# ericbill21/map-dit

Hardware: AMD Instinct MI355X
Metric: latent-images/sec training step, DiT-B/2 bf16 @256 (higher is better)
Workload: dtype bf16; 1 GPU; DiT-B/2 full training step on 32x32x4 latents (fresh batch+fwd+loss+bwd+grad reduction+Adam+2xEMA), all magnitude-preserving features on, bf16 GEMM operands / fp32 accumulate, master and residual fp32; global_batch=256, per_gpu_batch=256, parallelism=dp1, grad_comm=allreduce-fp32-per-stage-overlapped

## Files before the change

include/mapdit.h:

```cpp
#ifndef MAPDIT_H
#define MAPDIT_H

#include <stddef.h>
#include <stdint.h>

#ifdef __cplusplus
extern "C" {
#endif

#define MAPDIT_OK 0
#define MAPDIT_ERR_ARG 1
#define MAPDIT_ERR_HIP 2

const char* mapdit_last_error(void);
int mapdit_abi_version(void);

enum { MAPDIT_NT = 0, MAPDIT_NN = 1, MAPDIT_TN = 2 };

enum {
    MAPDIT_EPI_STORE_BF16 = 0,
    MAPDIT_EPI_STORE_F32 = 1,
    MAPDIT_EPI_SILU2 = 2,
    MAPDIT_EPI_RESID = 3,
    MAPDIT_EPI_DSILU = 4,
    MAPDIT_EPI_SILU2_COND = 5,
    MAPDIT_EPI_SILU2_GRAD = 7,
    MAPDIT_EPI_MUL_AUX = 8,
    MAPDIT_EPI_RMB = 9,
    MAPDIT_EPI_QKV_HEADS = 6,
    MAPDIT_EPI_QKV_HEADS_RAW = 10
};

typedef struct {
    int kind;
    void* out;
    int ldo;
    void* out2;
    const void* aux;
    const float* gate;
    int ldg;
    int rows_per_sample;
    float alpha, beta;
    int accumulate;
    void* out3;
    const float* shift2;
    const float* scale2;
    const float* gain2;
    int ld2;
    int split_k;
    long slab_stride;
    void* out4;
    const void* rmb;
    int rot2;
} mapdit_epilogue_t;

int mapdit_gemm_bf16(int layout, int M, int N, int K, const uint16_t* A, int lda, const uint16_t* B, int ldb,
                     const mapdit_epilogue_t* epi, void* stream);
typedef struct {
    const uint16_t* A; int lda;
    const uint16_t* B; int ldb;
    int M, N;
    float* out; int ldo;
    float alpha;
    long slab_stride;
} mapdit_gemm_group_item_t;
int mapdit_gemm_group_tn_bf16(int n, const mapdit_gemm_group_item_t* items, int K, int split_k, void* stream);
int mapdit_gemm_tile_size(int M, int N);
int mapdit_gemm_tile_size_ex(int M, int N, int split_k_launch);
int mapdit_gemm_tile_size_k(int M, int N, int K, int split_k_launch);
void mapdit_gemm_tuning(int tile, int phases, long band);

enum { MAPDIT_WN_PLAIN = 2 };
int mapdit_weightnorm_fwd(float* W, int rows, int cols, int forced, float out_scale, uint16_t* w_bf16, float* w_f32,
                          float* inv, void* stream);
typedef struct {
    float* W;
    int rows, cols;
    float out_scale;
    int first_block;
    uint16_t* w_bf16;
    float* w_f32;
    uint16_t* w_split3;
    int flags;
} mapdit_wn_job_t;
int mapdit_weightnorm_fwd_batch(const mapdit_wn_job_t* jobs_dev, int njobs, int total_blocks, int forced, void* stream);
int mapdit_weightnorm_bwd(const float* W, float* G, int ldg, int nslabs, long slab_stride, float* dW, int rows,
                          int cols, float out_scale, int accumulate, void* stream);
int mapdit_weightnorm_bwd_batch(const mapdit_wn_job_t* jobs_dev, int njobs, int total_blocks, void* stream);
typedef struct {
    const float* W; float* G; int ldg; int nslabs; long slab_stride; float* dW; int rows, cols; float out_scale; int flags;
} mapdit_wn_bwd_item_t;
int mapdit_weightnorm_bwd_group(int n, const mapdit_wn_bwd_item_t* items, void* stream);
int mapdit_weightnorm_bwd_slim(const float* W, float* G, int ldg, int nslabs, long slab_stride, float* dW, int rows,
                               int cols, float out_scale, int accumulate, void* stream);

typedef struct {
    long lo, hi, first_block;
} mapdit_range_t;

int mapdit_adam_ema_step(float* params, const float* grads, float* exp_avg, float* exp_avg_sq, float* ema_a,
                         float* ema_b, long n, const float* hyper, float beta1, float beta2, float eps, void* stream);
typedef struct {
    float step_size;
    float inv_sqrt_bc2;
    float ema_beta_a, ema_beta_b;
    float grad_scale;
} mapdit_adam_scalars_t;
int mapdit_adam_ema_step_scalars(float* params, const float* grads, float* exp_avg, float* exp_avg_sq, float* ema_a,
                                 float* ema_b, long n, const mapdit_adam_scalars_t* hyper, float beta1, float beta2,
                                 float eps, void* stream);
int mapdit_grad_nonfinite_check(const float* grads, long n, int* status, int step, void* stream);
int mapdit_adam_ema_step_guarded(float* params, const float* grads, float* exp_avg, float* exp_avg_sq, float* ema_a, float* ema_b,
                                 long n, const mapdit_adam_scalars_t* hyper, float beta1, float beta2, float eps,
                                 const int* status, int step, void* stream);
int mapdit_adam_ema_step_ranges(float* params, const float* grads, float* exp_avg, float* exp_avg_sq, float* ema_a, float* ema_b,
                                const mapdit_range_t* ranges_dev, int nranges, long total_blocks, const mapdit_adam_scalars_t* hyper,
                                float beta1, float beta2, float eps, const int* status, int step, void* stream);
int mapdit_grad_nonfinite_check_ranges(const float* grads, const mapdit_range_t* ranges_dev, int nranges, long total_blocks, int* status,
                                       int step, void* stream);

int mapdit_modulate_fwd(const float* x, const float* shift, const float* scale, int ldmod, const float* gain,
                        uint16_t* out, int n_samples, int T, int D, void* stream);

int mapdit_ln_modulate_fwd(const float* x, const float* shift, const float* scale, int ldmod, const float* gain, float* xhat, float* rstd,
                           uint16_t* out, int n_samples, int T, int D, void* stream);
int mapdit_ln_bwd_merge(const float* dxhat, const float* xhat, const float* rstd, const float* dxo, const uint16_t* dxo16, float ca, float* out,
                        long rows, int D, void* stream);

typedef struct {
    const float* dxo;
    const uint16_t* dxm;
    const float* x;
    const float* shift;
    const float* scale;
    const float* gain;
    const uint16_t* y_up;
    const float* g_up;
    float* dx;
    uint16_t* dx_bf;
    float* dshift;
    float* dscale;
    float* dgain_part;
    uint16_t* dy_up;
    float* dg_up;
    int ldmod, ldg_up, ldd, ldd_up;
    int n_samples, T, D;
    float ca, cb;
    float* part_scratch;
    size_t part_scratch_bytes;
    int* gain_partials_out;
    float* dgain_out;
    int rot;
    float dgain_scale;
    const uint16_t* dxo_bf;
    int ldx;
} mapdit_resid_mod_bwd_t;
int mapdit_resid_mod_bwd(const mapdit_resid_mod_bwd_t* args, void* stream);

int mapdit_rot_coef_fwd(const float* theta, const float* scale, int ldm, const float* gain, float* A, float* B, int ldc,
                        int n_samples, int D, void* stream);
#define MAPDIT_ROT_MAX_SLOTS 80
int mapdit_rot_coef_fwd_all(const float* mod, int ld_mod, const int* theta_off, const int* scale_off, const float* const* gains,
                            int n_slots, float* A, float* B, int ldc, int n_samples, int D, void* stream);
int mapdit_rot_coef_bwd(const float* dA, const float* dB, int ldc, const float* theta, const float* scale, int ldm,
                        const float* gain, float* dtheta, float* dscale, int ldd, float* dgain_part, float dgain_scale,
                        int n_samples, int D, void* stream);
int mapdit_rot_modulate_fwd(const float* x, const float* A, const float* B, int ldc, uint16_t* out, int n_samples, int T, int D,
                            void* stream);
int mapdit_reduce_partials(const float* part, int count, float* out, int accumulate, void* stream);

int mapdit_mpsilu_to_bf16(const float* x, uint16_t* out, long n, void* stream);
int mapdit_f32_to_bf16(const float* x, uint16_t* out, long n, float alpha, void* stream);
int mapdit_f32_to_bf16_2d(const float* x, int ldx, uint16_t* out, int ldo, int rows, int cols, float alpha, void* stream);
int mapdit_sum_slabs(float* acc, const float* slabs, int nslabs, long slab_stride, long n, void* stream);
int mapdit_reduce_slabs(float* out, const float* slabs, int nslabs, long slab_stride, long n, void* stream);
int mapdit_reduce_slabs_group(int n, float* const* outs, const float* const* slabs, const long* slab_strides, const long* ns, int nslabs, void* stream);
int mapdit_sum_bf16_chunks(float* out, const uint16_t* chunks, int nchunks, long chunk_stride, long n, void* stream);
int mapdit_scale_copy(float* out, const float* x, long n, float alpha, void* stream);

int mapdit_qkv_split(const uint16_t* qkv, int B, int T, int H, int head_dim, uint16_t* qn, uint16_t* kn, uint16_t* v,
                     void* stream);
int mapdit_qkv_merge_bwd(const uint16_t* qkv, int B, int T, int H, int head_dim, const uint16_t* dqn,
                         const uint16_t* dkn, const uint16_t* dv, uint16_t* dqkv, void* stream);
int mapdit_attn_cos_fwd(const uint16_t* qn, const uint16_t* kn, const uint16_t* v, uint16_t* o, float* lse, int B,
                        int T, int H, int head_dim, void* stream);
int mapdit_attn_cos_fwd_rawqk(const uint16_t* q, const uint16_t* k, const uint16_t* v, uint16_t* o, float* lse, int B, int T, int H,
                              int head_dim, void* stream);
int mapdit_attn_cos_fwd_rawqk_save(uint16_t* q, uint16_t* k, const uint16_t* v, uint16_t* o, float* lse, float* scales, int B, int T,
                                   int H, int head_dim, void* stream);
int mapdit_qk_cos_normalize(uint16_t* q, uint16_t* k, float* scales, int B, int T, int H, int head_dim, void* stream);
int mapdit_attn_sdpa_fwd(const uint16_t* q, const uint16_t* k, const uint16_t* v, uint16_t* o, float* lse, int B, int T, int H,
                         int head_dim, void* stream);
int mapdit_heads_merge_bwd(const uint16_t* dqn, const uint16_t* dkn, const uint16_t* dv, int B, int T, int H, int head_dim, uint16_t* dqkv,
                           void* stream);
int mapdit_attn_cos_bwd(const uint16_t* qn, const uint16_t* kn, const uint16_t* v, const uint16_t* dO, const uint16_t* O,
                        const float* lse, float* delta, uint16_t* dqn, uint16_t* dkn, uint16_t* dv, int B, int T, int H,
                        int head_dim, void* stream);
int mapdit_attn_cos_bwd_fused(const uint16_t* qn, const uint16_t* kn, const uint16_t* v, const uint16_t* dO, const uint16_t* O,
                              const float* lse, float* delta, const float* scales, uint16_t* dqkv, int B, int T, int H,
                              int head_dim, void* stream);

int mapdit_qkv_split_generic(const uint16_t* qkv, int B, int T, int H, int head_dim, uint16_t* qn, uint16_t* kn, uint16_t* v,
                             void* stream);
int mapdit_qkv_merge_bwd_generic(const uint16_t* qkv, int B, int T, int H, int head_dim, const uint16_t* dqn,
                                 const uint16_t* dkn, const uint16_t* dv, uint16_t* dqkv, void* stream);
int mapdit_attn_generic_fwd(const uint16_t* qn, const uint16_t* kn, const uint16_t* v, uint16_t* o, float* lse, int B, int T,
                            int H, int head_dim, void* stream);
int mapdit_attn_generic_bwd(const uint16_t* qn, const uint16_t* kn, const uint16_t* v, const uint16_t* dO, const uint16_t* O,
                            const float* lse, float* delta, uint16_t* dqn, uint16_t* dkn, uint16_t* dv, int B, int T, int H,
                            int head_dim, void* stream);

int mapdit_patch_embed_fwd(const float* x, const float* w_eff, const float* pos, float* out, uint16_t* patches,
                           int ldp, int N, int C, int S, int p, int D, float out_scale, void* stream);
int mapdit_patch_embed_bwd_x(const uint16_t* dx0, int ldx, const float* w_eff, float* dx, int N, int C, int S, int p, int D, float scale,
                             void* stream);
int mapdit_fourier_fwd(const int64_t* t, const float* scale, const float* shift, uint16_t* out, int n, int F,
                       void* stream);
int mapdit_cond_combine_fwd(const float* temb, const float* table, const int64_t* y, float* c, uint16_t* c_silu,
                            uint16_t* c_bf, int n, int D, int table_rows, void* stream);
int mapdit_cond_combine_bwd(const float* c, const float* dcs, const float* dcd, const int64_t* y, uint16_t* dtemb,
                            float* dtable, int n, int D, int table_rows, void* stream);
int mapdit_device_error_poll(void* stream);
int mapdit_final_out_fwd(const float* lin, int ldl, const float* a_mean, const float* a_sigma, const float* ref_mean,
                         const float* ref_sigma, float* out, int N, int C, int S, int p, void* stream);
int mapdit_final_out_bwd(const float* dout, const float* lin, int ldl, const float* a_mean, const float* a_sigma,
                         const float* ref_mean, const float* ref_sigma, uint16_t* dlin, int ldd, uint16_t* da_bf,
                         float* dref_part , float* dref_mean , float* dref_sigma,
                         float grad_scale, int N, int C, int S, int p, void* stream);
int mapdit_cfg_combine(const float* model_out, float* out, int n_total, int C, int HW, float cfg_scale, void* stream);
int mapdit_cfg_combine_bwd(const float* dout, float* din, int n_total, int C, int HW, float cfg_scale, void* stream);

int mapdit_q_sample(const float* x0, const float* noise, const int64_t* t, const float* tab, int nsteps, float* xt,
                    int N, int per_sample, void* stream);
int mapdit_loss_fwd(const float* model_out, const float* x0, const float* xt, const float* noise, const int64_t* t,
                    const float* tab, int nsteps, float* mse, float* vb, float* loss, float* G, int N, int per_sample,
                    void* stream);
int mapdit_loss_bwd(const float* G, const float* g_loss, const float* g_mse, const float* g_vb, float* dout, int N,
                    int per_sample, void* stream);
int mapdit_psample_step(const float* model_out, const float* x, const float* noise, const int64_t* t, const float* tab,
                        int nsteps, int clip_denoised, float* sample, float* pred_xstart, int N, int per_sample,
                        void* stream);
int mapdit_ddim_step(const float* model_out, const float* x, const float* noise, const int64_t* t, const float* tab,
                     const float* dtab, int nsteps, int clip_denoised, float eta, int reverse, float* sample, float* pred_xstart,
                     int N, int per_sample, void* stream);

int mapdit_obj_loss_fwd(const float* model_out, const float* x0, const float* xt, const float* noise, const int64_t* t,
                        const float* tab, const float* otab, int nsteps, int mean_type, int var_type, int loss_type, float* mse,
                        float* vb, float* loss, float* G, int N, int per_sample, void* stream);
int mapdit_obj_loss_bwd(const float* G, const float* g_loss, const float* g_mse, const float* g_vb, float* dout, int N,
                        int per_sample, int groups, void* stream);
int mapdit_obj_step(const float* model_out, const float* x, const float* noise, const int64_t* t, const float* tab,
                    const float* otab, int nsteps, int mean_type, int var_type, int clip_denoised, int mode, float eta,
                    float* sample, float* pred_xstart, int N, int per_sample, void* stream);
int mapdit_obj_xstart(const float* model_out, const float* x, const int64_t* t, const float* tab, int nsteps, int mean_type,
                      int var_type, float* xstart, int N, int per_sample, void* stream);
int mapdit_obj_step_guided(const float* model_out, const float* x, const float* noise, const int64_t* t, const float* tab,
                           const float* otab, int nsteps, int mean_type, int var_type, int clip_denoised, int mode, float eta,
                           const float* xstart_in, const float* cond_grad, float* sample, float* pred_xstart, float* mean, int N,
                           int per_sample, void* stream);
int mapdit_dpm_step(const float* model_out, const float* x, float* hist, const int64_t* step, const float* ctab, const int64_t* tau,
                    int K, const float* tab, int nsteps, int mean_type, int var_type, int clip_denoised, const float* xstart_in,
                    float* sample, float* pred_xstart, int N, int per_sample, void* stream);
int mapdit_obj_vb_terms(const float* model_out, const float* x0, const float* xt, const float* noise, const int64_t* t,
                        const float* tab, const float* otab, int nsteps, int mean_type, int var_type, int clip_denoised, float* vb,
                        float* xstart_mse, float* mse, float* pred_xstart, int ld, int col_from_t, int N, int per_sample,
                        void* stream);
int mapdit_prior_bpd(const float* x0, const float* tab, const float* otab, int nsteps, const float* vb, float* prior, float* total,
                     int N, int per_sample, void* stream);

enum { MAPDIT_OFF_MP_SILU = 1, MAPDIT_OFF_MP_RESIDUAL = 2, MAPDIT_OFF_MP_POS_ENC = 4, MAPDIT_OFF_MP_EMBEDDING = 8,
       MAPDIT_OFF_WEIGHT_NORM = 16, MAPDIT_OFF_COSINE_ATTN = 32, MAPDIT_OFF_NO_LAYERNORM = 64 };
typedef struct {
    int depth, hidden, patch, input_size, in_channels, num_heads, mlp_hidden;
    int table_rows;
    int max_batch;
    int precision;
    int rotation;
    int mp_off;
    float loss_scale;
    int recompute;
} mapdit_config_t;
enum { MAPDIT_RECOMPUTE_NONE = 0, MAPDIT_RECOMPUTE_MLP = 1, MAPDIT_RECOMPUTE_BLOCK = 2 };
enum { MAPDIT_PREC_BF16 = 0, MAPDIT_PREC_BF16X3 = 1, MAPDIT_PREC_F16 = 2 };

enum {
    MAPDIT_P_X_EMB = 0, MAPDIT_P_T0, MAPDIT_P_T2, MAPDIT_P_Y_EMB, MAPDIT_P_F_LIN, MAPDIT_P_F_MOD, MAPDIT_P_MS_LIN,
    MAPDIT_P_MS_REF, MAPDIT_P_SS_LIN, MAPDIT_P_SS_REF, MAPDIT_P_F_GAIN, MAPDIT_P_FOURIER_SCALE, MAPDIT_P_FOURIER_SHIFT,
    MAPDIT_P_POS_EMBED, MAPDIT_NUM_GLOBAL
};
enum { MAPDIT_B_QKV = 0, MAPDIT_B_PROJ, MAPDIT_B_FC1, MAPDIT_B_FC2, MAPDIT_B_MOD, MAPDIT_B_GAIN_MSA, MAPDIT_B_GAIN_MLP, MAPDIT_NUM_BLOCK };

typedef struct mapdit_engine mapdit_engine_t;

size_t mapdit_engine_workspace_bytes(const mapdit_config_t* cfg, int train);
int mapdit_engine_create(const mapdit_config_t* cfg, int train, void* workspace, size_t workspace_bytes, void* stream,
                         mapdit_engine_t** out);
void mapdit_engine_destroy(mapdit_engine_t* e);
int mapdit_engine_bind(mapdit_engine_t* e, float* const* params_host, float* const* grads_host);
int mapdit_engine_prepare_weights(mapdit_engine_t* e, int forced, void* stream);
int mapdit_engine_forward(mapdit_engine_t* e, const float* x, const int64_t* t, const int64_t* y_eff, int N, int save,
                          float* out, void* stream);
int mapdit_engine_backward(mapdit_engine_t* e, const float* dout, void* stream);
int mapdit_engine_backward_stages(mapdit_engine_t* e, const float* dout, int stage_from, int stage_to, void* stream);
int mapdit_engine_set_shard(mapdit_engine_t* e, int rank, int world);
int mapdit_engine_set_block_fences(mapdit_engine_t* e, void* const* events, int n);
int mapdit_engine_weight_image(mapdit_engine_t* e, int pidx, void** img, void** img3, int* rows, int* cols, int* sharded);
int mapdit_engine_jacobian_shard(mapdit_engine_t* e, void* stream);
int mapdit_engine_set_loss_scale(mapdit_engine_t* e, float loss_scale);
int mapdit_engine_loss_scale(mapdit_engine_t* e, float* out);
int mapdit_engine_set_input_grad(mapdit_engine_t* e, float* dx, int input_only);

enum { MAPDIT_PROF_FC1_FWD = 0 };
int mapdit_engine_profile_begin(mapdit_engine_t* e, int which, int max_events);
int mapdit_engine_profile_begin_strided(mapdit_engine_t* e, int which, int max_events, int stride);
int mapdit_engine_profile_end(mapdit_engine_t* e, int* count, double* total_ms);

enum { MAPDIT_PEEK_G_FOUR = 0, MAPDIT_PEEK_G_TEMB, MAPDIT_PEEK_G_C, MAPDIT_PEEK_G_MOD_ALL, MAPDIT_PEEK_G_X0, MAPDIT_PEEK_G_XMODF,
       MAPDIT_PEEK_G_LIN, MAPDIT_PEEK_B_XM, MAPDIT_PEEK_B_QKV, MAPDIT_PEEK_B_QN, MAPDIT_PEEK_B_KN, MAPDIT_PEEK_B_V, MAPDIT_PEEK_B_O,
       MAPDIT_PEEK_B_XM2, MAPDIT_PEEK_B_HACT, MAPDIT_PEEK_B_XMID, MAPDIT_PEEK_B_XOUT, MAPDIT_PEEK_COUNT };
int mapdit_engine_peek(mapdit_engine_t* e, int what, int block, void** ptr, long* elems, int* ld, int* dtype);

typedef struct mapdit_comm mapdit_comm_t;
int mapdit_comm_unique_id(void* id128);
int mapdit_comm_create(const void* id128, int rank, int world, mapdit_comm_t** out);
void mapdit_comm_destroy(mapdit_comm_t* comm);
int mapdit_allreduce_bucket(mapdit_comm_t* comm, float* buf, long count, void* stream);
int mapdit_reduce_scatter_bucket(mapdit_comm_t* comm, float* buf, long count, void* stream);
int mapdit_allgather_bucket(mapdit_comm_t* comm, float* buf, long count, void* stream);

int mapdit_gemm_f16(int layout, int M, int N, int K, const uint16_t* A, int lda, const uint16_t* B, int ldb,
                    const mapdit_epilogue_t* epi, void* stream);
int mapdit_gemm_group_tn_f16(int n, const mapdit_gemm_group_item_t* items, int K, int split_k, void* stream);
int mapdit_weightnorm_fwd_f16(float* W, int rows, int cols, int forced, float out_scale, uint16_t* w_f16, float* w_f32,
                              float* inv, void* stream);
int mapdit_weightnorm_fwd_batch_f16(const mapdit_wn_job_t* jobs_dev, int njobs, int total_blocks, int forced, void* stream);
int mapdit_modulate_fwd_f16(const float* x, const float* shift, const float* scale, int ldmod, const float* gain,
                            uint16_t* out, int n_samples, int T, int D, void* stream);
int mapdit_resid_mod_bwd_f16(const mapdit_resid_mod_bwd_t* args, void* stream);
int mapdit_ln_modulate_fwd_f16(const float* x, const float* shift, const float* scale, int ldmod, const float* gain, float* xhat, float* rstd,
                               uint16_t* out, int n_samples, int T, int D, void* stream);
int mapdit_ln_bwd_merge_f16(const float* dxhat, const float* xhat, const float* rstd, const float* dxo, const uint16_t* dxo16, float ca, float* out,
                            long rows, int D, void* stream);
int mapdit_rot_modulate_fwd_f16(const float* x, const float* A, const float* B, int ldc, uint16_t* out, int n_samples, int T, int D,
                                void* stream);
int mapdit_mpsilu_to_f16(const float* x, uint16_t* out, long n, void* stream);
int mapdit_f32_to_f16(const float* x, uint16_t* out, long n, float alpha, void* stream);
int mapdit_f32_to_f16_2d(const float* x, int ldx, uint16_t* out, int ldo, int rows, int cols, float alpha, void* stream);
int mapdit_qkv_split_f16(const uint16_t* qkv, int B, int T, int H, int head_dim, uint16_t* qn, uint16_t* kn, uint16_t* v,
                         void* stream);
int mapdit_qkv_merge_bwd_f16(const uint16_t* qkv, int B, int T, int H, int head_dim, const uint16_t* dqn,
                             const uint16_t* dkn, const uint16_t* dv, uint16_t* dqkv, void* stream);
int mapdit_attn_cos_fwd_f16(const uint16_t* qn, const uint16_t* kn, const uint16_t* v, uint16_t* o, float* lse, int B,
                            int T, int H, int head_dim, void* stream);
int mapdit_attn_cos_fwd_rawqk_f16(const uint16_t* q, const uint16_t* k, const uint16_t* v, uint16_t* o, float* lse, int B, int T, int H,
                                  int head_dim, void* stream);
int mapdit_attn_cos_fwd_rawqk_save_f16(uint16_t* q, uint16_t* k, const uint16_t* v, uint16_t* o, float* lse, float* scales, int B, int T,
                                       int H, int head_dim, void* stream);
int mapdit_qk_cos_normalize_f16(uint16_t* q, uint16_t* k, float* scales, int B, int T, int H, int head_dim, void* stream);
int mapdit_attn_sdpa_fwd_f16(const uint16_t* q, const uint16_t* k, const uint16_t* v, uint16_t* o, float* lse, int B, int T, int H,
                             int head_dim, void* stream);
int mapdit_heads_merge_bwd_f16(const uint16_t* dqn, const uint16_t* dkn, const uint16_t* dv, int B, int T, int H, int head_dim, uint16_t* dqkv,
                               void* stream);
int mapdit_attn_cos_bwd_f16(const uint16_t* qn, const uint16_t* kn, const uint16_t* v, const uint16_t* dO, const uint16_t* O,
                            const float* lse, float* delta, uint16_t* dqn, uint16_t* dkn, uint16_t* dv, int B, int T, int H,
                            int head_dim, void* stream);
int mapdit_attn_cos_bwd_fused_f16(const uint16_t* qn, const uint16_t* kn, const uint16_t* v, const uint16_t* dO, const uint16_t* O,
                                  const float* lse, float* delta, const float* scales, uint16_t* dqkv, int B, int T, int H,
                                  int head_dim, void* stream);
int mapdit_qkv_split_generic_f16(const uint16_t* qkv, int B, int T, int H, int head_dim, uint16_t* qn, uint16_t* kn, uint16_t* v,
                                 void* stream);
int mapdit_qkv_merge_bwd_generic_f16(const uint16_t* qkv, int B, int T, int H, int head_dim, const uint16_t* dqn,
                                     const uint16_t* dkn, const uint16_t* dv, uint16_t* dqkv, void* stream);
int mapdit_attn_generic_fwd_f16(const uint16_t* qn, const uint16_t* kn, const uint16_t* v, uint16_t* o, float* lse, int B, int T,
                                int H, int head_dim, void* stream);
int mapdit_attn_generic_bwd_f16(const uint16_t* qn, const uint16_t* kn, const uint16_t* v, const uint16_t* dO, const uint16_t* O,
                                const float* lse, float* delta, uint16_t* dqn, uint16_t* dkn, uint16_t* dv, int B, int T, int H,
                                int head_dim, void* stream);
int mapdit_patch_embed_fwd_f16(const float* x, const float* w_eff, const float* pos, float* out, uint16_t* patches,
                               int ldp, int N, int C, int S, int p, int D, float out_scale, void* stream);
int mapdit_patch_embed_bwd_x_f16(const uint16_t* dx0, int ldx, const float* w_eff, float* dx, int N, int C, int S, int p, int D, float scale,
                                 void* stream);
int mapdit_cond_combine_fwd_f16(const float* temb, const float* table, const int64_t* y, float* c, uint16_t* c_silu,
                                uint16_t* c_f16, int n, int D, int table_rows, void* stream);
int mapdit_cond_combine_bwd_f16(const float* c, const float* dcs, const float* dcd, const int64_t* y, uint16_t* dtemb,
                                float* dtable, int n, int D, int table_rows, void* stream);
int mapdit_final_out_bwd_f16(const float* dout, const float* lin, int ldl, const float* a_mean, const float* a_sigma,
                             const float* ref_mean, const float* ref_sigma, uint16_t* dlin, int ldd, uint16_t* da_f16,
                             float* dref_part, float* dref_mean, float* dref_sigma, float grad_scale, int N, int C, int S, int p,
                             void* stream);

#ifdef __cplusplus
}
#endif
#endif
```

map-dit_amd/_lib.py:

```python
from __future__ import annotations

import ctypes as C
import os
import subprocess
import threading

_HERE = os.path.dirname(os.path.abspath(__file__))
LIB_PATH = os.environ.get("MAPDIT_LIB") or os.path.join(_HERE, "libmapdit_hip.so")
CSRC = os.path.join(_HERE, "csrc")

vp, ci, cf, cl = C.c_void_p, C.c_int, C.c_float, C.c_long


class MapditError(RuntimeError):
    pass


class Epilogue(C.Structure):
    _fields_ = [("kind", ci), ("out", vp), ("ldo", ci), ("out2", vp), ("aux", vp), ("gate", vp), ("ldg", ci),
                ("rows_per_sample", ci), ("alpha", cf), ("beta", cf), ("accumulate", ci), ("out3", vp), ("shift2", vp), ("scale2", vp),
                ("gain2", vp), ("ld2", ci), ("split_k", ci), ("slab_stride", cl), ("out4", vp), ("rmb", vp), ("rot2", ci)]


class ResidModBwd(C.Structure):
    _fields_ = [("dxo", vp), ("dxm", vp), ("x", vp), ("shift", vp), ("scale", vp), ("gain", vp), ("y_up", vp),
                ("g_up", vp), ("dx", vp), ("dx_bf", vp), ("dshift", vp), ("dscale", vp), ("dgain_part", vp),
                ("dy_up", vp), ("dg_up", vp), ("ldmod", ci), ("ldg_up", ci), ("ldd", ci), ("ldd_up", ci),
                ("n_samples", ci), ("T", ci), ("D", ci), ("ca", cf), ("cb", cf), ("part_scratch", vp), ("part_scratch_bytes", C.c_size_t),
                ("gain_partials_out", C.POINTER(ci)), ("dgain_out", vp), ("rot", ci), ("dgain_scale", cf), ("dxo_bf", vp), ("ldx", ci)]


class GemmGroupItem(C.Structure):
    _fields_ = [("A", vp), ("lda", ci), ("B", vp), ("ldb", ci), ("M", ci), ("N", ci), ("out", vp), ("ldo", ci), ("alpha", cf), ("slab_stride", cl)]


class WnBwdItem(C.Structure):
    _fields_ = [("W", vp), ("G", vp), ("ldg", ci), ("nslabs", ci), ("slab_stride", cl), ("dW", vp), ("rows", ci), ("cols", ci), ("out_scale", cf),
                ("flags", ci)]


class WnJob(C.Structure):
    _fields_ = [("W", vp), ("rows", ci), ("cols", ci), ("out_scale", cf), ("first_block", ci), ("w_bf16", vp), ("w_f32", vp),
                ("w_split3", vp), ("flags", ci)]


class AdamScalars(C.Structure):
    _fields_ = [("step_size", cf), ("inv_sqrt_bc2", cf), ("ema_beta_a", cf), ("ema_beta_b", cf), ("grad_scale", cf)]


class Config(C.Structure):
    _fields_ = [("depth", ci), ("hidden", ci), ("patch", ci), ("input_size", ci), ("in_channels", ci),
                ("num_heads", ci), ("mlp_hidden", ci), ("table_rows", ci), ("max_batch", ci), ("precision", ci), ("rotation", ci),
                ("mp_off", ci), ("loss_scale", cf), ("recompute", ci)]


MP_OFF = {"mp_silu": 1, "mp_residual": 2, "mp_pos_enc": 4, "mp_embedding": 8, "weight_normalization": 16, "cosine_attention": 32, "no_layernorm": 64}
WN_PLAIN = 2


PRECISIONS = {"bf16": 0, "bf16x3": 1, "f16": 2}

RECOMPUTE = {"none": 0, "mlp": 1, "block": 2}


NT, NN, TN = 0, 1, 2
EPI_STORE_BF16, EPI_STORE_F32, EPI_SILU2, EPI_RESID, EPI_DSILU, EPI_SILU2_COND, EPI_QKV_HEADS, EPI_SILU2_GRAD, EPI_MUL_AUX, EPI_RMB, EPI_QKV_HEADS_RAW = range(11)
PROF_FC1_FWD = 0
PEEK_IDS = {name: i for i, name in enumerate(
    ["four", "temb", "c", "mod_all", "x0", "xmodf", "lin", "xm", "qkv", "qn", "kn", "v", "o", "xm2", "hact", "xmid", "xout"])}

(P_X_EMB, P_T0, P_T2, P_Y_EMB, P_F_LIN, P_F_MOD, P_MS_LIN, P_MS_REF, P_SS_LIN, P_SS_REF, P_F_GAIN, P_FOURIER_SCALE,
 P_FOURIER_SHIFT, P_POS_EMBED, NUM_GLOBAL) = range(15)
(B_QKV, B_PROJ, B_FC1, B_FC2, B_MOD, B_GAIN_MSA, B_GAIN_MLP, NUM_BLOCK) = range(8)

_SIGS = {
    "mapdit_gemm_bf16": [ci, ci, ci, ci, vp, ci, vp, ci, C.POINTER(Epilogue), vp],
    "mapdit_gemm_group_tn_bf16": [ci, vp, ci, ci, vp],
    "mapdit_weightnorm_fwd": [vp, ci, ci, ci, cf, vp, vp, vp, vp],
    "mapdit_weightnorm_bwd": [vp, vp, ci, ci, cl, vp, ci, ci, cf, ci, vp],
    "mapdit_weightnorm_bwd_slim": [vp, vp, ci, ci, cl, vp, ci, ci, cf, ci, vp],
    "mapdit_weightnorm_bwd_batch": [vp, ci, ci, vp],
    "mapdit_weightnorm_bwd_group": [ci, vp, vp],
    "mapdit_reduce_slabs_group": [ci, vp, vp, vp, vp, ci, vp],
    "mapdit_weightnorm_fwd_batch": [vp, ci, ci, ci, vp],
    "mapdit_adam_ema_step": [vp, vp, vp, vp, vp, vp, cl, vp, cf, cf, cf, vp],
    "mapdit_adam_ema_step_scalars": [vp, vp, vp, vp, vp, vp, cl, C.POINTER(AdamScalars), cf, cf, cf, vp],
    "mapdit_adam_ema_step_guarded": [vp, vp, vp, vp, vp, vp, cl, C.POINTER(AdamScalars), cf, cf, cf, vp, ci, vp],
    "mapdit_grad_nonfinite_check": [vp, cl, vp, ci, vp],
    "mapdit_adam_ema_step_ranges": [vp, vp, vp, vp, vp, vp, vp, ci, cl, C.POINTER(AdamScalars), cf, cf, cf, vp, ci, vp],
    "mapdit_grad_nonfinite_check_ranges": [vp, vp, ci, cl, vp, ci, vp],
    "mapdit_modulate_fwd": [vp, vp, vp, ci, vp, vp, ci, ci, ci, vp],
    "mapdit_resid_mod_bwd": [C.POINTER(ResidModBwd), vp],
    "mapdit_reduce_partials": [vp, ci, vp, ci, vp],
    "mapdit_rot_coef_fwd": [vp, vp, ci, vp, vp, vp, ci, ci, ci, vp],
    "mapdit_rot_coef_fwd_all": [vp, ci, vp, vp, vp, ci, vp, vp, ci, ci, ci, vp],
    "mapdit_rot_coef_bwd": [vp, vp, ci, vp, vp, ci, vp, vp, vp, ci, vp, cf, ci, ci, vp],
    "mapdit_rot_modulate_fwd": [vp, vp, vp, ci, vp, ci, ci, ci, vp],
    "mapdit_mpsilu_to_bf16": [vp, vp, cl, vp],
    "mapdit_f32_to_bf16": [vp, vp, cl, cf, vp],
    "mapdit_f32_to_bf16_2d": [vp, ci, vp, ci, ci, ci, cf, vp],
    "mapdit_sum_slabs": [vp, vp, ci, cl, cl, vp],
    "mapdit_scale_copy": [vp, vp, cl, cf, vp],
    "mapdit_reduce_slabs": [vp, vp, ci, cl, cl, vp],
    "mapdit_sum_bf16_chunks": [vp, vp, ci, cl, cl, vp],
    "mapdit_qkv_split": [vp, ci, ci, ci, ci, vp, vp, vp, vp],
    "mapdit_qkv_merge_bwd": [vp, ci, ci, ci, ci, vp, vp, vp, vp, vp],
    "mapdit_attn_cos_fwd": [vp, vp, vp, vp, vp, ci, ci, ci, ci, vp],
    "mapdit_attn_sdpa_fwd": [vp, vp, vp, vp, vp, ci, ci, ci, ci, vp],
    "mapdit_ln_modulate_fwd": [vp, vp, vp, ci, vp, vp, vp, vp, ci, ci, ci, vp],
    "mapdit_ln_bwd_merge": [vp, vp, vp, vp, vp, cf, vp, cl, ci, vp],
    "mapdit_heads_merge_bwd": [vp, vp, vp, ci, ci, ci, ci, vp, vp],
    "mapdit_attn_cos_fwd_rawqk": [vp, vp, vp, vp, vp, ci, ci, ci, ci, vp],
    "mapdit_attn_cos_fwd_rawqk_save": [vp, vp, vp, vp, vp, vp, ci, ci, ci, ci, vp],
    "mapdit_qk_cos_normalize": [vp, vp, vp, ci, ci, ci, ci, vp],
    "mapdit_attn_cos_bwd": [vp] * 10 + [ci, ci, ci, ci, vp],
    "mapdit_attn_cos_bwd_fused": [vp] * 9 + [ci, ci, ci, ci, vp],
    "mapdit_qkv_split_generic": [vp, ci, ci, ci, ci, vp, vp, vp, vp],
    "mapdit_qkv_merge_bwd_generic": [vp, ci, ci, ci, ci, vp, vp, vp, vp, vp],
    "mapdit_attn_generic_fwd": [vp, vp, vp, vp, vp, ci, ci, ci, ci, vp],
    "mapdit_attn_generic_bwd": [vp] * 10 + [ci, ci, ci, ci, vp],
    "mapdit_patch_embed_fwd": [vp, vp, vp, vp, vp, ci, ci, ci, ci, ci, ci, cf, vp],
    "mapdit_patch_embed_bwd_x": [vp, ci, vp, vp, ci, ci, ci, ci, ci, cf, vp],
    "mapdit_fourier_fwd": [vp, vp, vp, vp, ci, ci, vp],
    "mapdit_cond_combine_fwd": [vp, vp, vp, vp, vp, vp, ci, ci, ci, vp],
    "mapdit_cond_combine_bwd": [vp, vp, vp, vp, vp, vp, ci, ci, ci, vp],
    "mapdit_device_error_poll": [vp],
    "mapdit_comm_unique_id": [vp],
    "mapdit_comm_create": [vp, ci, ci, C.POINTER(vp)],
    "mapdit_allreduce_bucket": [vp, vp, cl, vp],
    "mapdit_reduce_scatter_bucket": [vp, vp, cl, vp],
    "mapdit_allgather_bucket": [vp, vp, cl, vp],
    "mapdit_final_out_fwd": [vp, ci, vp, vp, vp, vp, vp, ci, ci, ci, ci, vp],
    "mapdit_final_out_bwd": [vp, vp, ci, vp, vp, vp, vp, vp, ci, vp, vp, vp, vp, cf, ci, ci, ci, ci, vp],
    "mapdit_cfg_combine": [vp, vp, ci, ci, ci, cf, vp],
    "mapdit_cfg_combine_bwd": [vp, vp, ci, ci, ci, cf, vp],
    "mapdit_q_sample": [vp, vp, vp, vp, ci, vp, ci, ci, vp],
    "mapdit_loss_fwd": [vp, vp, vp, vp, vp, vp, ci, vp, vp, vp, vp, ci, ci, vp],
    "mapdit_loss_bwd": [vp, vp, vp, vp, vp, ci, ci, vp],
    "mapdit_psample_step": [vp, vp, vp, vp, vp, ci, ci, vp, vp, ci, ci, vp],
    "mapdit_ddim_step": [vp, vp, vp, vp, vp, vp, ci, ci, cf, ci, vp, vp, ci, ci, vp],
    "mapdit_obj_loss_fwd": [vp, vp, vp, vp, vp, vp, vp, ci, ci, ci, ci, vp, vp, vp, vp, ci, ci, vp],
    "mapdit_obj_loss_bwd": [vp, vp, vp, vp, vp, ci, ci, ci, vp],
    "mapdit_obj_step": [vp, vp, vp, vp, vp, vp, ci, ci, ci, ci, ci, cf, vp, vp, ci, ci, vp],
    "mapdit_obj_xstart": [vp, vp, vp, vp, ci, ci, ci, vp, ci, ci, vp],
    "mapdit_obj_step_guided": [vp, vp, vp, vp, vp, vp, ci, ci, ci, ci, ci, cf, vp, vp, vp, vp, vp, ci, ci, vp],
    "mapdit_dpm_step": [vp, vp, vp, vp, vp, vp, ci, vp, ci, ci, ci, ci, vp, vp, vp, ci, ci, vp],
    "mapdit_obj_vb_terms": [vp, vp, vp, vp, vp, vp, vp, ci, ci, ci, ci, vp, vp, vp, vp, ci, ci, ci, ci, vp],
    "mapdit_prior_bpd": [vp, vp, vp, ci, vp, vp, vp, ci, ci, vp],
    "mapdit_engine_create": [C.POINTER(Config), ci, vp, C.c_size_t, vp, C.POINTER(vp)],
    "mapdit_engine_bind": [vp, C.POINTER(vp), C.POINTER(vp)],
    "mapdit_engine_prepare_weights": [vp, ci, vp],
    "mapdit_engine_forward": [vp, vp, vp, vp, ci, ci, vp, vp],
    "mapdit_engine_backward": [vp, vp, vp],
    "mapdit_engine_backward_stages": [vp, vp, ci, ci, vp],
    "mapdit_engine_set_shard": [vp, ci, ci],
    "mapdit_engine_set_block_fences": [vp, C.POINTER(vp), ci],
    "mapdit_engine_weight_image": [vp, ci, C.POINTER(vp), C.POINTER(vp), C.POINTER(ci), C.POINTER(ci), C.POINTER(ci)],
    "mapdit_engine_jacobian_shard": [vp, vp],
    "mapdit_engine_set_loss_scale": [vp, cf],
    "mapdit_engine_loss_scale": [vp, C.POINTER(cf)],
    "mapdit_engine_set_input_grad": [vp, vp, ci],
    "mapdit_engine_profile_begin": [vp, ci, ci],
    "mapdit_engine_profile_begin_strided": [vp, ci, ci, ci],
    "mapdit_engine_profile_end": [vp, C.POINTER(ci), C.POINTER(C.c_double)],
    "mapdit_engine_peek": [vp, ci, ci, C.POINTER(vp), C.POINTER(C.c_long), C.POINTER(ci), C.POINTER(ci)],
}
for _n in ("weightnorm_fwd", "weightnorm_fwd_batch", "modulate_fwd", "resid_mod_bwd", "rot_modulate_fwd", "qkv_split",
           "qkv_merge_bwd", "attn_cos_fwd", "attn_cos_fwd_rawqk", "attn_cos_fwd_rawqk_save", "qk_cos_normalize", "attn_cos_bwd", "attn_cos_bwd_fused", "attn_sdpa_fwd", "heads_merge_bwd", "ln_modulate_fwd", "ln_bwd_merge", "qkv_split_generic", "qkv_merge_bwd_generic",
           "attn_generic_fwd", "attn_generic_bwd", "patch_embed_fwd", "patch_embed_bwd_x", "cond_combine_fwd", "cond_combine_bwd", "final_out_bwd"):
    _SIGS[f"mapdit_{_n}_f16"] = _SIGS[f"mapdit_{_n}"]
for _b, _h in (("gemm_bf16", "gemm_f16"), ("gemm_group_tn_bf16", "gemm_group_tn_f16"), ("f32_to_bf16", "f32_to_f16"), ("f32_to_bf16_2d", "f32_to_f16_2d"),
               ("mpsilu_to_bf16", "mpsilu_to_f16")):
    _SIGS[f"mapdit_{_h}"] = _SIGS[f"mapdit_{_b}"]
_OTHER = {
    "mapdit_last_error": (C.c_char_p, []),
    "mapdit_abi_version": (ci, []),
    "mapdit_gemm_tile_size": (ci, [ci, ci]),
    "mapdit_gemm_tile_size_ex": (ci, [ci, ci, ci]),
    "mapdit_gemm_tile_size_k": (ci, [ci, ci, ci, ci]),
    "mapdit_gemm_tuning": (None, [ci, ci, cl]),
    "mapdit_engine_workspace_bytes": (C.c_size_t, [C.POINTER(Config), ci]),
    "mapdit_engine_destroy": (None, [vp]),
    "mapdit_comm_destroy": (None, [vp]),
}
EXPORTS = sorted(list(_SIGS) + list(_OTHER))

_lock = threading.Lock()
_handle = None


def _source_digest() -> str:
    import hashlib
    h = hashlib.sha256()
    inc = os.path.join(os.path.dirname(_HERE), "include", "mapdit.h")
    files = sorted(os.path.join(CSRC, f) for f in os.listdir(CSRC) if f.endswith((".hip", ".h")) or f == "Makefile") + [inc]
    for f in files:
        h.update(os.path.basename(f).encode() + b"\0")
        with open(f, "rb") as fh:
            h.update(fh.read())
    return h.hexdigest()


def build(force: bool = False) -> str:
    stamp = LIB_PATH + ".src-sha256"
    digest = _source_digest()
    if not force and os.path.exists(LIB_PATH) and os.path.exists(stamp) and open(stamp).read().strip() == digest:
        return LIB_PATH
    if force:
        subprocess.check_call(["make", "-C", CSRC, "clean"])
    subprocess.check_call(["make", "-C", CSRC, "-j8"])
    with open(stamp, "w") as f:
        f.write(digest + "\n")
    return LIB_PATH


class _Lib:
    def __init__(self, cdll):
        self._cdll = cdll
        for name, argtypes in _SIGS.items():
            fn = getattr(cdll, name)
            fn.argtypes = argtypes
            fn.restype = ci
            setattr(self, name[len("mapdit_"):], self._wrap(name, fn))
        for name, (res, argtypes) in _OTHER.items():
            fn = getattr(cdll, name)
            fn.argtypes = argtypes
            fn.restype = res
            setattr(self, name[len("mapdit_"):], fn)

    def _wrap(self, name, fn):
        def call(*args):
            rc = fn(*args)
            if rc != 0:
                raise MapditError(f"{name} failed ({rc}): {self._cdll.mapdit_last_error().decode()}")
        call.__name__ = name
        return call


def lib() -> _Lib:
    global _handle
    with _lock:
        if _handle is None:
            if not os.path.exists(LIB_PATH):
                raise MapditError(f"{LIB_PATH} is missing: run `python -c 'import __graft_entry__ as g; g.build()'` "
                                  f"or `make -C {CSRC}`; there is no CPU fallback")
            import torch
            _handle = _Lib(C.CDLL(LIB_PATH))
        return _handle


def ptr(t):
    return None if t is None else t.data_ptr()


def cur_stream():
    import torch
    return torch.cuda.current_stream().cuda_stream
```

map-dit_amd/csrc/gemm.hip:

```cpp
#include <stdarg.h>
#include <type_traits>
#include <stdio.h>

#include "common.h"

MD_NS_OPEN

constexpr int BM = 128, BN = 128, BKT = 64;
constexpr int TILE_BYTES = 16384;
constexpr int BUF_BYTES = 2 * TILE_BYTES;
constexpr int CS_LD = 132;
constexpr int SMEM_BYTES = BM * CS_LD * 4;

enum { OP_ROW = 0, OP_KMAJ = 1 };

struct GemmP {
    const bf16_t* A;
    const bf16_t* B;
    int lda, ldb;
    int M, N, K;
    int tiles_n;
    int tiles;
    int split_k;
    int band;
    int phases;
    int n_off;
    int stagger;
};

__device__ __forceinline__ int kswz(int k) { return (k & 3) | ((k >> 1) & 4); }

__device__ __attribute__((aligned(16))) const unsigned int g_zero16[4] = {0u, 0u, 0u, 0u};

template <int KIND, bool KTAIL>
__device__ __forceinline__ void stage_tile(const bf16_t* __restrict__ G, int ld, int idx0, int idx_max, int k0, int kmax,
                                           char* tile, int wave, int lane) {
#pragma unroll
    for (int j = 0; j < 4; ++j) {
        const int seg = wave * 4 + j;
        const bf16_t* src;
        if (KIND == OP_ROW) {
            const int row = seg * 8 + (lane >> 3);
            const int c = (lane & 7) ^ (row & 7);
            int grow = idx0 + row;
            grow = grow < idx_max ? grow : idx_max - 1;
            src = G + (size_t)grow * ld + k0 + c * 8;
            if (KTAIL && k0 + c * 8 >= kmax) src = (const bf16_t*)g_zero16;
        } else {
            const int krow = seg * 4 + (lane >> 4);
            const int c = (lane & 15) ^ (kswz(krow) << 1);
            int col = idx0 + c * 8;
            col = col < idx_max ? col : 0;
            src = G + (size_t)(k0 + krow) * ld + col;
            if (KTAIL && k0 + krow >= kmax) src = (const bf16_t*)g_zero16;
        }
        __builtin_amdgcn_global_load_lds(src, (lds_void_t*)(tile + seg * 1024), 16, 0, 0);
    }
}

template <int KIND, bool TR_ASM = true>
__device__ __forceinline__ bf16x8_t read_frag(const char* tile, int i0, int ks, int lane) {
    if (KIND == OP_ROW) {
        const int row = i0 + (lane & 15);
        const int c = 4 * ks + (lane >> 4);
        return *(const bf16x8_t*)(tile + row * 128 + ((c ^ (row & 7)) << 4));
    } else {
        const int g = lane >> 4, i = lane & 15, q = i >> 2, pp = i & 3;
        const int c = (i0 >> 3) + (pp >> 1);
        const int sub = (pp & 1) << 3;
        bf16x4_t lo, hi;
        if constexpr (!TR_ASM) {
            const int k_a = 32 * ks + 8 * g + q, k_b = k_a + 4;
            const int off_a = k_a * 256 + ((c ^ (kswz(k_a) << 1)) << 4) + sub;
            const int off_b = k_b * 256 + ((c ^ (kswz(k_b) << 1)) << 4) + sub;
            typedef __attribute__((address_space(3))) bf16x4_t lds_v4;
            lo = __builtin_amdgcn_ds_read_tr16_b64_v4i16((lds_v4*)(tile + off_a));
            hi = __builtin_amdgcn_ds_read_tr16_b64_v4i16((lds_v4*)(tile + off_b));
        } else {
        const int k0 = 8 * g + q;
        const unsigned addr = (unsigned)(size_t)(const __attribute__((address_space(3))) char*)(tile + k0 * 256 + ((c ^ (kswz(k0) << 1)) << 4) + sub);
        if (ks == 0)
            asm volatile("ds_read_b64_tr_b16 %0, %2\n\tds_read_b64_tr_b16 %1, %2 offset:1024" : "=&v"(lo), "=&v"(hi) : "v"(addr));
        else
            asm volatile("ds_read_b64_tr_b16 %0, %2 offset:8192\n\tds_read_b64_tr_b16 %1, %2 offset:9216" : "=&v"(lo), "=&v"(hi) : "v"(addr));
        }
        bf16x8_t r;
        r[0] = lo[0]; r[1] = lo[1]; r[2] = lo[2]; r[3] = lo[3];
        r[4] = hi[0]; r[5] = hi[1]; r[6] = hi[2]; r[7] = hi[3];
        return r;
    }
}

struct EpiNoAux {};
struct EpiNoTile {};
typedef __attribute__((ext_vector_type(2))) unsigned int u32x2_t;
template <class Epi> constexpr int kDirectOuts = 0;
typedef __attribute__((ext_vector_type(4))) unsigned int u32x4_t;
__device__ __forceinline__ void store16_stream(void* p, u32x4_t v, bool keep = false) {
    if (keep) *(u32x4_t*)p = v;
    else __builtin_nontemporal_store(v, (u32x4_t*)p);
}
__device__ __forceinline__ void store8_bf16(bf16_t* p, const float* v, bool keep = false) {
    u32x4_t u;
    u.x = pack16(v[0], v[1]); u.y = pack16(v[2], v[3]); u.z = pack16(v[4], v[5]); u.w = pack16(v[6], v[7]);
    store16_stream(p, u, keep);
}
__device__ __forceinline__ void load8_bf16(const bf16_t* p, float* v) {
    const u32x4_t u = __builtin_nontemporal_load((const u32x4_t*)p);
    v[0] = lo16(u.x); v[1] = hi16(u.x);
    v[2] = lo16(u.y); v[3] = hi16(u.y);
    v[4] = lo16(u.z); v[5] = hi16(u.z);
    v[6] = lo16(u.w); v[7] = hi16(u.w);
}

template <bool U, class T> __device__ __forceinline__ T* rowptr(T* p, int m, int n, int ld, unsigned off) {
    if constexpr (U) return (T*)((char*)(p + (size_t)m * ld + n) + (size_t)off * sizeof(T));
    else return p + (size_t)m * ld + n;
}
__device__ __forceinline__ int opaque_s(int x) { asm volatile("" : "+s"(x)); return x; }
template <class Epi> constexpr bool kUniformRows = false;

#define EPI_TRIVIAL_STEPS                                                                                      \
    typedef EpiNoAux Aux;                                                                                      \
    typedef EpiNoTile Tile;                                                                                    \
    __device__ __forceinline__ Tile tile_begin(int, int, int) const { return Tile(); }                         \
    __device__ __forceinline__ Aux load(int, int) const { return Aux(); }                                      \
    __device__ __forceinline__ void apply(int m, int n, const float* v, int z, const Aux&, const Tile&) const { (*this)(m, n, v, z); }
struct EpiStoreBf16 {
    bf16_t* out; int ldo; float alpha; int keep;
    EPI_TRIVIAL_STEPS
    __device__ __forceinline__ int n_direct() const { return 1; }
    __device__ __forceinline__ bool keep_direct() const { return keep != 0; }
    __device__ __forceinline__ bf16_t* dst(int) const { return out; }
    __device__ __forceinline__ void pw(const f32x4_t& v, u32x2_t* o, int) const {
        o[0] = u32x2_t{pack16(alpha * v[0], alpha * v[1]), pack16(alpha * v[2], alpha * v[3])};
    }
    __device__ __forceinline__ void operator()(int m, int n, const float* v, int = 0) const {
        float w[8];
#pragma unroll
        for (int i = 0; i < 8; ++i) w[i] = alpha * v[i];
        store8_bf16(out + (size_t)m * ldo + n, w, keep);
    }
};
struct EpiStoreF32 {
    float* out; int ldo; float alpha; int accumulate; long slab_stride;
    EPI_TRIVIAL_STEPS
    __device__ __forceinline__ void operator()(int m, int n, const float* v, int z = 0) const {
        float4* p = (float4*)(out + (size_t)z * slab_stride + (size_t)m * ldo + n);
        float4 a = make_float4(alpha * v[0], alpha * v[1], alpha * v[2], alpha * v[3]);
        float4 b = make_float4(alpha * v[4], alpha * v[5], alpha * v[6], alpha * v[7]);
        if (accumulate) {
            float4 x = p[0], y = p[1];
            a.x += x.x; a.y += x.y; a.z += x.z; a.w += x.w;
            b.x += y.x; b.y += y.y; b.z += y.z; b.w += y.w;
        }
        p[0] = a; p[1] = b;
    }
};
template <int TAG> struct EpiSilu2 {
    bf16_t* pre; bf16_t* act; int ldo;
    EPI_TRIVIAL_STEPS
    __device__ __forceinline__ void operator()(int m, int n, const float* v, int = 0) const {
        float a[8];
#pragma unroll
        for (int i = 0; i < 8; ++i) a[i] = silu_f(v[i]) * (1.f / MP_SILU_DIV);
        if (pre) store8_bf16(pre + (size_t)m * ldo + n, v);
        store8_bf16(act + (size_t)m * ldo + n, a);
    }
};
template <bool HAS_D> struct EpiSilu2GradT {
    bf16_t* dact; bf16_t* act; int ldo; int keep;
    __device__ __forceinline__ bool keep_direct() const { return false; }
    EPI_TRIVIAL_STEPS
    __device__ __forceinline__ int n_direct() const { return HAS_D ? 2 : 1; }
    __device__ __forceinline__ bf16_t* dst(int w) const { return w == 0 ? act : dact; }
    __device__ __forceinline__ void pw(const f32x4_t& v, u32x2_t* o, int nout) const {
        float a[4], d[4];
#pragma unroll
        for (int i = 0; i < 4; ++i) {
            const float s = __builtin_amdgcn_rcpf(1.f + __expf(-v[i]));
            a[i] = v[i] * s * (1.f / MP_SILU_DIV);
            d[i] = s * (1.f + v[i] * (1.f - s)) * (1.f / MP_SILU_DIV);
        }
        o[0] = u32x2_t{pack16(a[0], a[1]), pack16(a[2], a[3])};
        if (nout > 1) o[1] = u32x2_t{pack16(d[0], d[1]), pack16(d[2], d[3])};
    }
    __device__ __forceinline__ void operator()(int m, int n, const float* v, int = 0) const {
        typedef __attribute__((ext_vector_type(2))) float f2;
        float a[8], d[8];
#pragma unroll
        for (int i = 0; i < 8; i += 2) {
            const f2 x = {v[i], v[i + 1]};
            const f2 t = x * -1.44269504088896341f;
            const f2 e = {__builtin_amdgcn_exp2f(t.x), __builtin_amdgcn_exp2f(t.y)};
            const f2 q = e * MP_SILU_DIV + MP_SILU_DIV;
            const f2 sc = {__builtin_amdgcn_rcpf(q.x), __builtin_amdgcn_rcpf(q.y)};
            const f2 ac = x * sc;
            a[i] = ac.x; a[i + 1] = ac.y;
            if constexpr (HAS_D) {
                const f2 om = sc * -MP_SILU_DIV + 1.f;
                const f2 dd = ac * om + sc;
                d[i] = dd.x; d[i + 1] = dd.y;
            }
        }
        if constexpr (HAS_D) store8_bf16(dact + (size_t)m * ldo + n, d);
        store8_bf16(act + (size_t)m * ldo + n, a, keep != 0);
    }
};
template <> constexpr int kDirectOuts<EpiStoreBf16> = 1;
struct EpiMulAux {
    bf16_t* out; const bf16_t* aux; int ldo; int keep;
    struct Aux { u32x4_t h; };
    typedef EpiNoTile Tile;
    __device__ __forceinline__ Tile tile_begin(int, int, int) const { return Tile(); }
    __device__ __forceinline__ Aux load(int m, int n) const {
        Aux a; a.h = __builtin_nontemporal_load((const u32x4_t*)(aux + (size_t)m * ldo + n));
        return a;
    }
    __device__ __forceinline__ void apply(int m, int n, const float* v, int, const Aux& a, const Tile&) const {
        const u32x4_t u = a.h;
        float w[8];
        w[0] = v[0] * lo16(u.x); w[1] = v[1] * hi16(u.x);
        w[2] = v[2] * lo16(u.y); w[3] = v[3] * hi16(u.y);
        w[4] = v[4] * lo16(u.z); w[5] = v[5] * hi16(u.z);
        w[6] = v[6] * lo16(u.w); w[7] = v[7] * hi16(u.w);
        store8_bf16(out + (size_t)m * ldo + n, w, keep != 0);
    }
    __device__ __forceinline__ void operator()(int m, int n, const float* v, int = 0) const { apply(m, n, v, 0, load(m, n), Tile()); }
};
struct EpiResid {
    bf16_t* y; const float* xin; float* xout; const float* gate; int ldo, ldg, rows; float ca, cb;
    bf16_t* xm; const float* nshift; const float* nscale; const float* ngain; int ldn;
    int rot;
    int xm_plain;
    struct Aux { float4 x0, x1; };
    struct Tile { float4 g0, g1, c0, c1, h0, h1; float ka, kb; int smp; };
    __device__ __forceinline__ void per_sample(int smp, int n, Tile& t) const {
        const float4* g = (const float4*)(gate + (size_t)smp * ldg + n);
        t.g0 = g[0]; t.g1 = g[1];
        if (xm) {
            const float4* sc = (const float4*)(nscale + (size_t)smp * ldn + n);
            const float4* sh = (const float4*)(nshift + (size_t)smp * ldn + n);
            t.c0 = sc[0]; t.c1 = sc[1]; t.h0 = sh[0]; t.h1 = sh[1];
        }
    }
    __device__ __forceinline__ Tile tile_begin(int m_first, int m_last, int n) const {
        Tile t;
        t.smp = m_first / rows == m_last / rows ? m_first / rows : -1;
        t.ka = t.kb = 0.f;
        if (xm && !rot) {
            const float gg = *ngain, den = sqrtf((1.f - gg) * (1.f - gg) + gg * gg);
            t.ka = (1.f - gg) / den; t.kb = gg / den;
        }
        if (t.smp >= 0) per_sample(t.smp, n, t);
        return t;
    }
    __device__ __forceinline__ Aux load(int m, int n) const {
        const float4* xi = (const float4*)(xin + (size_t)m * ldo + n);
        Aux a; a.x0 = xi[0]; a.x1 = xi[1];
        return a;
    }
    bool fast_ok() const { return rows % 256 == 0 && xm_plain == 1 && y && xm && !rot; }
    __device__ __forceinline__ int ld_rows() const { return ldo; }
    __device__ __forceinline__ Aux load_u(int R, int n0u, unsigned off) const {
        const float4* xi = (const float4*)rowptr<true>(xin, R, n0u, ldo, off);
        Aux a; a.x0 = xi[0]; a.x1 = xi[1];
        return a;
    }
    template <bool ONE>
    __device__ __forceinline__ void apply_u(int R, int n0u, unsigned off, const float* v, int, const Aux& a, const Tile& tc) const {
        core<true, true>(R, n0u, off, v, a, tc);
    }
    __device__ __forceinline__ void apply(int m, int n, const float* v, int z, const Aux& a, const Tile& tc) const {
        apply_t<false>(m, n, v, z, a, tc);
    }
    template <bool ONE>
    __device__ __forceinline__ void apply_t(int m, int n, const float* v, int, const Aux& a, const Tile& tc) const {
        core<ONE, false>(m, n, 0u, v, a, tc);
    }
    template <bool ONE, bool U>
    __device__ __forceinline__ void core(int m, int n, unsigned off, const float* v, const Aux& a, const Tile& tc) const {
        Tile t = tc;
        if (!ONE && tc.smp < 0) per_sample(m / rows, n, t);
        const float g[8] = {t.g0.x, t.g0.y, t.g0.z, t.g0.w, t.g1.x, t.g1.y, t.g1.z, t.g1.w};
        const float x[8] = {a.x0.x, a.x0.y, a.x0.z, a.x0.w, a.x1.x, a.x1.y, a.x1.z, a.x1.w};
        float o[8];
#pragma unroll
        for (int i = 0; i < 8; ++i) o[i] = __builtin_fmaf(cb * g[i], v[i], ca * x[i]);
        if (!U && (xm_plain & 2)) {
            __builtin_nontemporal_store(f32x4_t{o[0], o[1], o[2], o[3]}, (f32x4_t*)rowptr<U>(xout, m, n, ldo, off));
            __builtin_nontemporal_store(f32x4_t{o[4], o[5], o[6], o[7]}, (f32x4_t*)rowptr<U>(xout, m, n, ldo, off) + 1);
        } else {
            float4* xo = (float4*)rowptr<U>(xout, m, n, ldo, off);
            xo[0] = make_float4(o[0], o[1], o[2], o[3]);
            xo[1] = make_float4(o[4], o[5], o[6], o[7]);
        }
        if (U || y) store8_bf16(rowptr<U>(y, m, n, ldo, off), v);
        if (U || xm) {
            const float c[8] = {t.c0.x, t.c0.y, t.c0.z, t.c0.w, t.c1.x, t.c1.y, t.c1.z, t.c1.w};
            const float h[8] = {t.h0.x, t.h0.y, t.h0.z, t.h0.w, t.h1.x, t.h1.y, t.h1.z, t.h1.w};
            float w[8];
            if (!U && rot) {
#pragma unroll
                for (int i = 0; i < 8; ++i) w[i] = __builtin_fmaf(o[i], c[i], o[i ^ 1] * h[i]);
            } else {
#pragma unroll
                for (int i = 0; i < 8; ++i) w[i] = __builtin_fmaf(t.ka * o[i], c[i], t.kb * h[i]);
            }
#pragma unroll
            for (int i = 0; i < 8; ++i) asm volatile("" : "+v"(w[i]));
            store8_bf16(rowptr<U>(xm, m, n, ldo, off), w, U || (xm_plain & 1) != 0);
        }
    }
    __device__ __forceinline__ void operator()(int m, int n, const float* v, int = 0) const {
        apply(m, n, v, 0, load(m, n), tile_begin(m, m, n));
    }
};
struct EpiDSilu {
    bf16_t* out; const bf16_t* pre; int ldo;
    struct Aux { u32x4_t h; };
    typedef EpiNoTile Tile;
    __device__ __forceinline__ Tile tile_begin(int, int, int) const { return Tile(); }
    __device__ __forceinline__ Aux load(int m, int n) const {
        Aux a; a.h = __builtin_nontemporal_load((const u32x4_t*)(pre + (size_t)m * ldo + n));
        return a;
    }
    __device__ __forceinline__ void apply(int m, int n, const float* v, int, const Aux& a, const Tile&) const {
        const u32x4_t u = a.h;
        float h[8], w[8];
        h[0] = lo16(u.x); h[1] = hi16(u.x);
        h[2] = lo16(u.y); h[3] = hi16(u.y);
        h[4] = lo16(u.z); h[5] = hi16(u.z);
        h[6] = lo16(u.w); h[7] = hi16(u.w);
#pragma unroll
        for (int i = 0; i < 8; ++i) w[i] = v[i] * dmpsilu_f(h[i]);
        store8_bf16(out + (size_t)m * ldo + n, w);
    }
    __device__ __forceinline__ void operator()(int m, int n, const float* v, int = 0) const {
        float h[8], w[8];
        load8_bf16(pre + (size_t)m * ldo + n, h);
#pragma unroll
        for (int i = 0; i < 8; ++i) w[i] = v[i] * dmpsilu_f(h[i]);
        store8_bf16(out + (size_t)m * ldo + n, w);
    }
};

template <bool DX16, bool FAST = false> struct EpiRmbT {
    const bf16_t* dxo16;
    const float* dxo; const float* x; const float* shift; const float* scale; const float* gain;
    const bf16_t* y_up; const float* g_up;
    float* dx; bf16_t* dx_bf; bf16_t* dy_up; float* dshift; float* dscale; float* dg_up; float* dgain_part;
    int ldo, ldmod, ldg_up, ldd, ldd_up, T; float ca, cb, gscale;
    struct AuxF { float4 x0, x1, d0, d1; u32x4_t y, d16; };
    struct AuxH { float4 x0, x1; u32x4_t y, d16; };
    typedef typename std::conditional<DX16, AuxH, AuxF>::type Aux;
    struct Tile { float4 sc0, sc1, sh0, sh1, gu0, gu1; };
    struct Acc { float sc[8], sh[8], g[8], gain; };
    __device__ __forceinline__ void coef(float& k, float& kb, float& kd) const {
        const float gg = *gain, den = sqrtf((1.f - gg) * (1.f - gg) + gg * gg);
        k = (1.f - gg) / den; kb = gg / den; kd = 1.f / den;
    }
    __device__ __forceinline__ Tile block_begin(int m_block, int n) const {
        const int smp = m_block / T;
        Tile t;
        const float4* sc = (const float4*)(scale + (size_t)smp * ldmod + n);
        const float4* sh = (const float4*)(shift + (size_t)smp * ldmod + n);
        t.sc0 = sc[0]; t.sc1 = sc[1]; t.sh0 = sh[0]; t.sh1 = sh[1];
        t.gu0 = t.gu1 = make_float4(0.f, 0.f, 0.f, 0.f);
        if (FAST || y_up) {
            const float4* gu = (const float4*)(g_up + (size_t)smp * ldg_up + n);
            t.gu0 = gu[0]; t.gu1 = gu[1];
        }
        return t;
    }
    __device__ __forceinline__ Aux load(int m, int n) const {
        Aux a;
        const float4* xi = (const float4*)(x + (size_t)m * ldo + n);
        a.x0 = xi[0]; a.x1 = xi[1];
        if constexpr (!DX16) a.d0 = a.d1 = make_float4(0.f, 0.f, 0.f, 0.f);
        a.d16 = u32x4_t{0u, 0u, 0u, 0u};
        if constexpr (FAST) {
            a.d16 = *(const u32x4_t*)(dxo16 + (size_t)m * ldo + n);
            a.y = __builtin_nontemporal_load((const u32x4_t*)(y_up + (size_t)m * ldo + n));
            return a;
        } else if constexpr (DX16) {
            if (dxo16) a.d16 = *(const u32x4_t*)(dxo16 + (size_t)m * ldo + n);
        } else {
            if (dxo) {
                const float4* di = (const float4*)(dxo + (size_t)m * ldo + n);
                a.d0 = di[0]; a.d1 = di[1];
            }
        }
        a.y = u32x4_t{0u, 0u, 0u, 0u};
        if (y_up) a.y = __builtin_nontemporal_load((const u32x4_t*)(y_up + (size_t)m * ldo + n));
        return a;
    }
    __device__ __forceinline__ void apply_r(int m, int n, const float* v, const Aux& a, const Tile& t, Acc& r, float k, float kb,
                                            float kd) const {

        const float xx[8] = {a.x0.x, a.x0.y, a.x0.z, a.x0.w, a.x1.x, a.x1.y, a.x1.z, a.x1.w};
        float dd[8];
        if constexpr (!DX16) {
            dd[0] = a.d0.x; dd[1] = a.d0.y; dd[2] = a.d0.z; dd[3] = a.d0.w; dd[4] = a.d1.x; dd[5] = a.d1.y; dd[6] = a.d1.z; dd[7] = a.d1.w;
        } else {
            dd[0] = lo16(a.d16.x); dd[1] = hi16(a.d16.x); dd[2] = lo16(a.d16.y); dd[3] = hi16(a.d16.y);
            dd[4] = lo16(a.d16.z); dd[5] = hi16(a.d16.z); dd[6] = lo16(a.d16.w); dd[7] = hi16(a.d16.w);
        }
        const float sc[8] = {t.sc0.x, t.sc0.y, t.sc0.z, t.sc0.w, t.sc1.x, t.sc1.y, t.sc1.z, t.sc1.w};
        const float sh[8] = {t.sh0.x, t.sh0.y, t.sh0.z, t.sh0.w, t.sh1.x, t.sh1.y, t.sh1.z, t.sh1.w};
        float o[8];
#pragma unroll
        for (int i = 0; i < 8; ++i) {
            const float vi = up16(cvt16(v[i]));
            o[i] = __builtin_fmaf(k * sc[i], vi, ca * dd[i]);
            r.sc[i] += k * xx[i] * vi;
            r.sh[i] += kb * vi;
            r.gain += vi * (sh[i] - xx[i] * sc[i]) * kd;
        }
#pragma unroll
        for (int i = 0; i < 8; ++i) asm volatile("" : "+v"(o[i]));
        if (!FAST && dx) {
            float4* p = (float4*)(dx + (size_t)m * ldo + n);
            p[0] = make_float4(o[0], o[1], o[2], o[3]);
            p[1] = make_float4(o[4], o[5], o[6], o[7]);
        }
        if (FAST || dx_bf) store8_bf16(dx_bf + (size_t)m * ldo + n, o);
        if (FAST || y_up) {
            const float gu[8] = {t.gu0.x, t.gu0.y, t.gu0.z, t.gu0.w, t.gu1.x, t.gu1.y, t.gu1.z, t.gu1.w};
            const u32x4_t u = a.y;
            const float yy[8] = {lo16(u.x), hi16(u.x), lo16(u.y),
                                 hi16(u.y), lo16(u.z), hi16(u.z),
                                 lo16(u.w), hi16(u.w)};
            float w[8];
#pragma unroll
            for (int i = 0; i < 8; ++i) {
                w[i] = cb * gu[i] * o[i];
                r.g[i] += cb * yy[i] * o[i];
            }
            store8_bf16(dy_up + (size_t)m * ldo + n, w);
        }
    }
    typedef EpiNoTile TileUnused;
    __device__ __forceinline__ void operator()(int, int, const float*, int = 0) const {}
};
template <> constexpr bool kUniformRows<EpiResid> = true;
template <bool ONE, class E> __device__ __forceinline__ void epi_apply_t(const E& e, int m, int n, const float* v, int z,
                                                                         const typename E::Aux& a, const typename E::Tile& t);
template <class E> __device__ __forceinline__ typename E::Aux epi_load_u(const E& e, int R, int n0u, unsigned off) {
    if constexpr (kUniformRows<E>) return e.load_u(opaque_s(R), n0u, off); else return typename E::Aux();
}
template <class E> __device__ __forceinline__ void epi_apply_u(const E& e, int R, int n0u, unsigned off, const float* v, int z,
                                                               const typename E::Aux& a, const typename E::Tile& t) {
    if constexpr (kUniformRows<E>) e.template apply_u<true>(opaque_s(R), n0u, off, v, z, a, t);
}
template <class Epi> constexpr bool kFastEpi = false;
template <> constexpr bool kFastEpi<EpiResid> = true;
template <class Epi> constexpr bool kOneSample = false;
template <> constexpr bool kOneSample<EpiResid> = true;
template <bool ONE, class E> __device__ __forceinline__ void epi_apply_t(const E& e, int m, int n, const float* v, int z,
                                                                         const typename E::Aux& a, const typename E::Tile& t) {
    if constexpr (kOneSample<E>) e.template apply_t<ONE>(m, n, v, z, a, t); else e.apply(m, n, v, z, a, t);
}
template <class Epi> constexpr bool kReduce = false;
template <> constexpr bool kReduce<EpiRmbT<false>> = true;
template <> constexpr bool kReduce<EpiRmbT<true>> = true;
template <> constexpr bool kReduce<EpiRmbT<true, true>> = true;

struct EpiQkvHeads {
    int keep;
    bf16_t *qn, *kn, *v; float* s; int T, H;
    long rows_total;
    int tshift;
    typedef EpiNoAux Aux;
    struct Tile { bf16_t* dst; float* sdst; int which, h, d; };
    __device__ __forceinline__ Tile tile_begin(int, int, int n) const {
        const int D = 64 * H;
        Tile t;
        t.which = n / D;
        const int c = n - t.which * D;
        t.h = c >> 6; t.d = c & 63;
        t.dst = (t.which == 0 ? qn : t.which == 1 ? kn : v) + t.d;
        t.sdst = s + (size_t)t.which * (size_t)rows_total;
        return t;
    }
    __device__ __forceinline__ Aux load(int, int) const { return Aux(); }
    __device__ __forceinline__ void apply(int m, int, const float* a, int, const Aux&, const Tile& tc) const {
        const int b = tshift >= 0 ? m >> tshift : m / T, t = m - b * T;
        const size_t row = ((size_t)b * H + tc.h) * T + t;
        float w[8];
        if (tc.which < 2) {
            float ss = 0.f;
#pragma unroll
            for (int i = 0; i < 8; ++i) ss += a[i] * a[i];
            ss = sum8(ss);
            const float sc = 8.f * __builtin_amdgcn_rcpf(__builtin_amdgcn_sqrtf(ss) + NORM_EPS);
#pragma unroll
            for (int i = 0; i < 8; ++i) w[i] = a[i] * sc;
            if (tc.d == 0) tc.sdst[row] = sc;
        } else {
#pragma unroll
            for (int i = 0; i < 8; ++i) w[i] = a[i];
        }
        store8_bf16(tc.dst + row * 64, w, keep != 0);
    }
    __device__ __forceinline__ void operator()(int m, int n, const float* a, int = 0) const {
        apply(m, n, a, 0, Aux(), tile_begin(m, m, n));
    }
};

struct EpiHeadsRaw {
    bf16_t *q, *k, *v; int T, H, hd;
    int tshift;
    typedef EpiNoAux Aux;
    struct Tile { bf16_t* dst; int h; };
    __device__ __forceinline__ Tile tile_begin(int, int, int n) const {
        const int D = hd * H, which = n / D, c = n - which * D;
        Tile t;
        t.h = c / hd;
        t.dst = (which == 0 ? q : which == 1 ? k : v) + (c - t.h * hd);
        return t;
    }
    __device__ __forceinline__ Aux load(int, int) const { return Aux(); }
    __device__ __forceinline__ void apply(int m, int, const float* a, int, const Aux&, const Tile& tc) const {
        const int b = tshift >= 0 ? m >> tshift : m / T, t = m - b * T;
        store8_bf16(tc.dst + (((size_t)b * H + tc.h) * T + t) * hd, a);
    }
    __device__ __forceinline__ void operator()(int m, int n, const float* a, int = 0) const {
        apply(m, n, a, 0, Aux(), tile_begin(m, m, n));
    }
};

template <int AK, int BK, class Epi, bool KTAIL = false>
__global__ __launch_bounds__(256, 2) void gemm_mfma_kernel(GemmP p, Epi epi) {
    __shared__ __attribute__((aligned(16))) char smem[SMEM_BYTES];
    const int tid = threadIdx.x, lane = tid & 63;
    const int wave = __builtin_amdgcn_readfirstlane(tid >> 6);
    const int wm = wave >> 1, wn = wave & 1;

    const int nwg = gridDim.x, bid = blockIdx.x;
    const int xcd = bid & 7, q = nwg >> 3, r = nwg & 7;
    const int wg = (xcd < r ? xcd * (q + 1) : r * (q + 1) + (xcd - r) * q) + (bid >> 3);
    const int z = wg / p.tiles, tile = wg - z * p.tiles;
    const int m0 = (tile / p.tiles_n) * BM, n0 = (tile % p.tiles_n) * BN;
    const int nkt = (p.K + BKT - 1) / BKT, kbase = nkt / p.split_k, krem = nkt % p.split_k;
    const int kbeg = (z * kbase + (z < krem ? z : krem)) * BKT;

    f32x4_t acc[4][4];
#pragma unroll
    for (int i = 0; i < 4; ++i)
#pragma unroll
        for (int j = 0; j < 4; ++j) acc[i][j] = f32x4_t{0.f, 0.f, 0.f, 0.f};

    const int nk = kbase + (z < krem ? 1 : 0);
    stage_tile<AK, KTAIL>(p.A, p.lda, m0, p.M, kbeg, p.K, smem, wave, lane);
    stage_tile<BK, KTAIL>(p.B, p.ldb, n0, p.N, kbeg, p.K, smem + TILE_BYTES, wave, lane);
    for (int t = 0; t < nk; ++t) {
        __syncthreads();
        char* cur = smem + (t & 1) * BUF_BYTES;
        if (t + 1 < nk) {
            char* nxt = smem + ((t + 1) & 1) * BUF_BYTES;
            stage_tile<AK, KTAIL>(p.A, p.lda, m0, p.M, kbeg + (t + 1) * BKT, p.K, nxt, wave, lane);
            stage_tile<BK, KTAIL>(p.B, p.ldb, n0, p.N, kbeg + (t + 1) * BKT, p.K, nxt + TILE_BYTES, wave, lane);
        }
#pragma unroll
        for (int ks = 0; ks < 2; ++ks) {
            bf16x8_t fa[4], fb[4];
#pragma unroll
            for (int i = 0; i < 4; ++i) fa[i] = read_frag<AK>(cur, wm * 64 + i * 16, ks, lane);
#pragma unroll
            for (int j = 0; j < 4; ++j) fb[j] = read_frag<BK>(cur + TILE_BYTES, wn * 64 + j * 16, ks, lane);
            if (AK == OP_KMAJ || BK == OP_KMAJ) {
                asm volatile("s_waitcnt lgkmcnt(0)" ::: "memory");
                __builtin_amdgcn_sched_barrier(0);
            }
#pragma unroll
            for (int i = 0; i < 4; ++i)
#pragma unroll
                for (int j = 0; j < 4; ++j)
                    acc[i][j] = MFMA16(fb[j], fa[i], acc[i][j]);
        }
    }
    __syncthreads();

    float* cs = (float*)smem;
#pragma unroll
    for (int i = 0; i < 4; ++i)
#pragma unroll
        for (int j = 0; j < 4; ++j) {
            const int m = wm * 64 + i * 16 + (lane & 15);
            const int n = wn * 64 + j * 16 + 4 * (lane >> 4);
            *(f32x4_t*)(cs + m * CS_LD + n) = acc[i][j];
        }
    __syncthreads();
#pragma unroll
    for (int it = 0; it < 8; ++it) {
        const int row = (tid >> 4) + 16 * it, col = (tid & 15) * 8;
        const int gm = m0 + row, gn = n0 + col;
        if (gm < p.M && gn < p.N) {
            float v[8];
            *(f32x4_t*)(v) = *(const f32x4_t*)(cs + row * CS_LD + col);
            *(f32x4_t*)(v + 4) = *(const f32x4_t*)(cs + row * CS_LD + col + 4);
            epi(gm, gn + p.n_off, v, z);
        }
    }
}

template <int BK, class Epi>
__global__ __launch_bounds__(256, 2) void gemm_mfma64_kernel(GemmP p, Epi epi) {
    __shared__ __attribute__((aligned(16))) char smem[SMEM_BYTES];
    const int tid = threadIdx.x, lane = tid & 63;
    const int wave = __builtin_amdgcn_readfirstlane(tid >> 6);
    const int nwg = gridDim.x, bid = blockIdx.x;
    const int xcd = bid & 7, q = nwg >> 3, r = nwg & 7;
    const int tile = (xcd < r ? xcd * (q + 1) : r * (q + 1) + (xcd - r) * q) + (bid >> 3);
    const int m0 = (tile / p.tiles_n) * 64, n0 = (tile % p.tiles_n) * BN;
    const int nk = p.K / BKT;
    f32x4_t acc[4][2];
#pragma unroll
    for (int i = 0; i < 4; ++i)
#pragma unroll
        for (int j = 0; j < 2; ++j) acc[i][j] = f32x4_t{0.f, 0.f, 0.f, 0.f};
    if (wave < 2) stage_tile<OP_ROW, false>(p.A, p.lda, m0, p.M, 0, p.K, smem, wave, lane);
    stage_tile<BK, false>(p.B, p.ldb, n0, p.N, 0, p.K, smem + TILE_BYTES, wave, lane);
    for (int t = 0; t < nk; ++t) {
        __syncthreads();
        char* cur = smem + (t & 1) * BUF_BYTES;
        if (t + 1 < nk) {
            char* nxt = smem + ((t + 1) & 1) * BUF_BYTES;
            if (wave < 2) stage_tile<OP_ROW, false>(p.A, p.lda, m0, p.M, (t + 1) * BKT, p.K, nxt, wave, lane);
            stage_tile<BK, false>(p.B, p.ldb, n0, p.N, (t + 1) * BKT, p.K, nxt + TILE_BYTES, wave, lane);
        }
#pragma unroll
        for (int ks = 0; ks < 2; ++ks) {
            bf16x8_t fa[4], fb[2];
#pragma unroll
            for (int i = 0; i < 4; ++i) fa[i] = read_frag<OP_ROW>(cur, i * 16, ks, lane);
#pragma unroll
            for (int j = 0; j < 2; ++j) fb[j] = read_frag<BK>(cur + TILE_BYTES, wave * 32 + j * 16, ks, lane);
            if (BK == OP_KMAJ) {
                asm volatile("s_waitcnt lgkmcnt(0)" ::: "memory");
                __builtin_amdgcn_sched_barrier(0);
            }
#pragma unroll
            for (int i = 0; i < 4; ++i)
#pragma unroll
                for (int j = 0; j < 2; ++j) acc[i][j] = MFMA16(fb[j], fa[i], acc[i][j]);
        }
    }
    __syncthreads();
    float* cs = (float*)smem;
#pragma unroll
    for (int i = 0; i < 4; ++i)
#pragma unroll
        for (int j = 0; j < 2; ++j) {
            const int m = i * 16 + (lane & 15);
            const int n = wave * 32 + j * 16 + 4 * (lane >> 4);
            *(f32x4_t*)(cs + m * CS_LD + n) = acc[i][j];
        }
    __syncthreads();
#pragma unroll
    for (int it = 0; it < 4; ++it) {
        const int row = (tid >> 4) + 16 * it, col = (tid & 15) * 8;
        const int gm = m0 + row, gn = n0 + col;
        if (gm < p.M && gn < p.N) {
            float v[8];
            *(f32x4_t*)(v) = *(const f32x4_t*)(cs + row * CS_LD + col);
            *(f32x4_t*)(v + 4) = *(const f32x4_t*)(cs + row * CS_LD + col + 4);
            epi(gm, gn + p.n_off, v, 0);
        }
    }
}

constexpr int BM2 = 256, BN2 = 256;
constexpr int SLOT_BYTES = 16384, KBUF_BYTES = 4 * SLOT_BYTES;
constexpr int OFF_A0 = 0, OFF_A1 = SLOT_BYTES, OFF_B0 = 2 * SLOT_BYTES, OFF_B1 = 3 * SLOT_BYTES;
constexpr int CS2_LD = 260;
constexpr int SMEM2_BYTES = 128 * CS2_LD * 4;
#ifdef MAPDIT_GEMM_STAMPS
constexpr int STAMP_TILES = 12, STAMP_POINTS = 11;
__device__ long long* g_stamps = nullptr;
__device__ long long* g_wg_times = nullptr;
extern "C" __global__ void mapdit_debug_set_wg_times_kernel(long long* p) { g_wg_times = p; }
__device__ int g_stamp_block = -1;
extern "C" __global__ void mapdit_debug_set_stamps_kernel(long long* p, int block) { g_stamps = p; g_stamp_block = block; }
#define G256_STAMP(PT)                                                                              \
    if (stamp_on && t < STAMP_TILES) {                                                              \
        __builtin_amdgcn_sched_barrier(0);                                                          \
        stamp_lds[(wm * STAMP_TILES + t) * STAMP_POINTS + (PT)] = (long long)__builtin_readcyclecounter(); \
        __builtin_amdgcn_sched_barrier(0);                                                          \
    }
#define G256_TSTAMP(IDX)                                                                            \
    if (wave == 0 && (IDX) < 3) {                        \
        __builtin_amdgcn_sched_barrier(0);                                                          \
        kl_[(IDX) % 3] = (long long)__builtin_readcyclecounter();                                       \
        __builtin_amdgcn_sched_barrier(0);                                                          \
    }                                                                                               \
    if (stamp_on && wave == 0) {                                                                    \
        __builtin_amdgcn_sched_barrier(0);                                                          \
        stamp_lds[2 * STAMP_TILES * STAMP_POINTS + (IDX)] = (long long)__builtin_readcyclecounter(); \
        __builtin_amdgcn_sched_barrier(0);                                                          \
    }
#define G256_RSTAMP(IDX)                                                                            \
    if (stamp_on && wave == 0) {                                                                    \
        __builtin_amdgcn_sched_barrier(0);                                                          \
        stamp_lds[2 * STAMP_TILES * STAMP_POINTS + (IDX)] = (long long)__builtin_amdgcn_s_memrealtime(); \
        __builtin_amdgcn_sched_barrier(0);                                                          \
    }
#define G256_STAMPS_OUT()                                                                           \
    if (g_wg_times && wave == 0 && lane == 0) {                                                     \
        long long* r_ = g_wg_times + 4 * (long long)bid;                                     \
        r_[0] = wg_r0; r_[1] = (long long)__builtin_amdgcn_s_memrealtime();                         \
        const long long now_ = (long long)__builtin_readcyclecounter();                             \
        r_[2] = now_ - wg_t0;                                                                       \
                       \
        r_[3] = ((long long)__builtin_amdgcn_s_getreg(((4 - 1) << 11) | (0 << 6) | 20) & 0xff) |    \
                (((kl_[2] - kl_[1]) & 0xffffff) << 8) | (((kl_[1] - wg_t0) & 0xffff) << 32) |       \
                (((now_ - kl_[2]) & 0xffff) << 48);                                                 \
    }                                                                                               \
    if (stamp_on) {                                                                                 \
        for (int i = 0; i < STAMP_TILES * STAMP_POINTS; ++i)                                        \
            g_stamps[wm * STAMP_TILES * STAMP_POINTS + i] = stamp_lds[wm * STAMP_TILES * STAMP_POINTS + i]; \
        if (wave == 0)                                                                              \
            for (int i = 0; i < 8; ++i) g_stamps[2 * STAMP_TILES * STAMP_POINTS + i] = stamp_lds[2 * STAMP_TILES * STAMP_POINTS + i]; \
    }
#else
#define G256_STAMP(PT)
#define G256_TSTAMP(IDX)
#define G256_RSTAMP(IDX)
#define G256_STAMPS_OUT()
#endif

template <int SIDE> __device__ __forceinline__ int half_map(int i, int h) {
    return SIDE == 0 ? ((i >> 6) * 128 + h * 64 + (i & 63)) : ((i >> 5) * 64 + h * 32 + (i & 31));
}

template <int KIND, int SIDE, bool KTAIL>
__device__ __forceinline__ void stage_half(const bf16_t* __restrict__ G, int ld, int idx0, int idx_max, int k0, int kmax, int h,
                                           char* slot, int wave, int lane) {
#pragma unroll
    for (int j = 0; j < 2; ++j) {
        const int seg = wave * 2 + j;
        const bf16_t* src;
        if (KIND == OP_ROW) {
            const int row = seg * 8 + (lane >> 3);
            const int c = (lane & 7) ^ (row & 7);
            int g = idx0 + half_map<SIDE>(row, h);
            g = g < idx_max ? g : idx_max - 1;
            src = G + (size_t)g * ld + k0 + c * 8;
            if (KTAIL && k0 + c * 8 >= kmax) src = (const bf16_t*)g_zero16;
        } else {
            const int krow = seg * 4 + (lane >> 4);
            const int c = (lane & 15) ^ (kswz(krow) << 1);
            int col = idx0 + half_map<SIDE>(c * 8, h);
            col = col < idx_max ? col : 0;
            src = G + (size_t)(k0 + krow) * ld + col;
            if (KTAIL && k0 + krow >= kmax) src = (const bf16_t*)g_zero16;
        }
        __builtin_amdgcn_global_load_lds(src, (lds_void_t*)(slot + seg * 1024), 16, 0, 0);
    }
}

#define G256_END_LOAD()                                   \
    asm volatile("s_waitcnt lgkmcnt(0)" ::: "memory");    \
    __builtin_amdgcn_sched_barrier(0);                    \
    __builtin_amdgcn_s_barrier();                         \
    __builtin_amdgcn_sched_barrier(0)
#define G256_END_MFMA()                                   \
    __builtin_amdgcn_sched_barrier(0);                    \
    __builtin_amdgcn_s_barrier();                         \
    __builtin_amdgcn_sched_barrier(0)

template <int AK, int BK, class Epi, bool KTAIL, bool FE = false>
__device__ __forceinline__ void gemm256_tile(const GemmP& p, const Epi& epi, char* smem, const int bid, const int nwg) {
#ifdef MAPDIT_GEMM_STAMPS
    long long* stamp_lds = (long long*)(smem + SMEM2_BYTES);
    const long long wg_t0 = (long long)__builtin_readcyclecounter();
    const long long wg_r0 = (long long)__builtin_amdgcn_s_memrealtime();
    long long kl_[3] = {0, 0, 0};
#endif
    int tid_ = threadIdx.x;
    asm volatile("" : "+v"(tid_));
    const int tid = tid_, lane = tid & 63;
    const int wave = __builtin_amdgcn_readfirstlane(tid >> 6);
    const int wm = wave >> 2, wn = wave & 3;
#ifdef MAPDIT_GEMM_STAMPS
    const bool stamp_on = g_stamps && bid == (g_stamp_block >= 0 ? g_stamp_block : 8) && (wave == 0 || wave == 4) && lane == 0;
#endif
    G256_TSTAMP(0);

    const int xcd = bid & 7, q = nwg >> 3, r = nwg & 7;
    const int wg = (xcd < r ? xcd * (q + 1) : r * (q + 1) + (xcd - r) * q) + (bid >> 3);
    const int z = wg / p.tiles, tile = wg - z * p.tiles;
    const int tiles_m = p.tiles / p.tiles_n;
    const int bsz = tiles_m * p.band;
    const int bidx = tile / bsz, rem = tile - bidx * bsz;
    const int bw = (bidx + 1) * p.band <= p.tiles_n ? p.band : p.tiles_n - bidx * p.band;
    const int m0 = (rem / bw) * BM2, n0 = (bidx * p.band + rem % bw) * BN2;
    const int nkt = (p.K + BKT - 1) / BKT, kbase = nkt / p.split_k, krem = nkt % p.split_k;
    const int kbeg = (z * kbase + (z < krem ? z : krem)) * BKT;
    const int nk = kbase + (z < krem ? 1 : 0);

    f32x4_t acc[8][4];
#pragma unroll
    for (int i = 0; i < 8; ++i)
#pragma unroll
        for (int j = 0; j < 4; ++j) acc[i][j] = f32x4_t{0.f, 0.f, 0.f, 0.f};
    bf16x8_t fa[4][2], fb0[2][2], fb1[2][2];
    constexpr bool TR_ASM2 = AK == OP_KMAJ;

    auto load_a = [&](const char* slot) {
#pragma unroll
        for (int i = 0; i < 4; ++i)
#pragma unroll
            for (int ks = 0; ks < 2; ++ks) fa[i][ks] = read_frag<AK, TR_ASM2>(slot, wm * 64 + i * 16, ks, lane);
    };
#define G256_LOAD_B(FB, SLOT)                                                                                  \
    _Pragma("unroll") for (int j = 0; j < 2; ++j)                                                              \
    _Pragma("unroll") for (int ks = 0; ks < 2; ++ks) FB[j][ks] = read_frag<BK, TR_ASM2>(SLOT, wn * 32 + j * 16, ks, lane)
#define G256_MFMA(MQ, NQ, FB)                                                                                  \
    __builtin_amdgcn_s_setprio(1);                                                                             \
    _Pragma("unroll") for (int ks = 0; ks < 2; ++ks)                                                           \
    _Pragma("unroll") for (int i = 0; i < 4; ++i)                                                              \
    _Pragma("unroll") for (int j = 0; j < 2; ++j)                                                              \
        acc[(MQ) * 4 + i][(NQ) * 2 + j] =                                                                      \
            MFMA16(FB[j][ks], fa[i][ks], acc[(MQ) * 4 + i][(NQ) * 2 + j]); \
    __builtin_amdgcn_s_setprio(0)
#define G256_WAIT_DMA(has2)                                                  \
    if (has2) asm volatile("s_waitcnt vmcnt(10)" ::: "memory");              \
    else asm volatile("s_waitcnt vmcnt(0)" ::: "memory")

    stage_half<AK, 0, KTAIL>(p.A, p.lda, m0, p.M, kbeg, p.K, 0, smem + OFF_A0, wave, lane);
    stage_half<BK, 1, KTAIL>(p.B, p.ldb, n0, p.N, kbeg, p.K, 0, smem + OFF_B0, wave, lane);
    stage_half<BK, 1, KTAIL>(p.B, p.ldb, n0, p.N, kbeg, p.K, 1, smem + OFF_B1, wave, lane);
    stage_half<AK, 0, KTAIL>(p.A, p.lda, m0, p.M, kbeg, p.K, 1, smem + OFF_A1, wave, lane);
    if (nk > 1) {
        char* b1 = smem + KBUF_BYTES;
        stage_half<AK, 0, KTAIL>(p.A, p.lda, m0, p.M, kbeg + BKT, p.K, 0, b1 + OFF_A0, wave, lane);
        stage_half<BK, 1, KTAIL>(p.B, p.ldb, n0, p.N, kbeg + BKT, p.K, 0, b1 + OFF_B0, wave, lane);
        stage_half<BK, 1, KTAIL>(p.B, p.ldb, n0, p.N, kbeg + BKT, p.K, 1, b1 + OFF_B1, wave, lane);
        if (p.phases == 2) asm volatile("s_waitcnt vmcnt(8)" ::: "memory");
        else asm volatile("s_waitcnt vmcnt(10)" ::: "memory");
    } else {
        asm volatile("s_waitcnt vmcnt(0)" ::: "memory");
    }
    __builtin_amdgcn_sched_barrier(0);
    __builtin_amdgcn_s_barrier();
    __builtin_amdgcn_sched_barrier(0);
    if (wm == 1) {
        __builtin_amdgcn_s_barrier();
        __builtin_amdgcn_sched_barrier(0);
    }

    G256_TSTAMP(1);
    G256_RSTAMP(5);
    if (p.phases == 2) {
        for (int t = 0; t < nk; ++t) {
            char* cur = smem + (t & 1) * KBUF_BYTES;
            char* nxt = smem + ((t + 1) & 1) * KBUF_BYTES;
            const int k1 = kbeg + (t + 1) * BKT, k2 = kbeg + (t + 2) * BKT;
            const bool has1 = t + 1 < nk, has2 = t + 2 < nk;
            G256_STAMP(0);
            load_a(cur + OFF_A0);
            G256_LOAD_B(fb0, cur + OFF_B0);
            G256_LOAD_B(fb1, cur + OFF_B1);
            if (has1) {
                stage_half<AK, 0, KTAIL>(p.A, p.lda, m0, p.M, k1, p.K, 1, nxt + OFF_A1, wave, lane);
                G256_STAMP(1);
                asm volatile("s_waitcnt vmcnt(8)" ::: "memory");
            } else {
                asm volatile("s_waitcnt vmcnt(0)" ::: "memory");
            }
            G256_STAMP(2);
            G256_END_LOAD();
            G256_STAMP(3);
            G256_MFMA(0, 0, fb0);
            G256_MFMA(0, 1, fb1);
            G256_STAMP(4);
            G256_END_MFMA();
            G256_STAMP(5);
            load_a(cur + OFF_A1);
            if (has2) {
                stage_half<AK, 0, KTAIL>(p.A, p.lda, m0, p.M, k2, p.K, 0, cur + OFF_A0, wave, lane);
                stage_half<BK, 1, KTAIL>(p.B, p.ldb, n0, p.N, k2, p.K, 0, cur + OFF_B0, wave, lane);
                stage_half<BK, 1, KTAIL>(p.B, p.ldb, n0, p.N, k2, p.K, 1, cur + OFF_B1, wave, lane);
                G256_STAMP(6);
                asm volatile("s_waitcnt vmcnt(8)" ::: "memory");
            } else if (has1) {
                asm volatile("s_waitcnt vmcnt(2)" ::: "memory");
            } else {
                asm volatile("s_waitcnt vmcnt(0)" ::: "memory");
            }
            G256_STAMP(7);
            G256_END_LOAD();
            G256_STAMP(8);
            G256_MFMA(1, 1, fb1);
            G256_MFMA(1, 0, fb0);
            G256_STAMP(9);
            G256_END_MFMA();
            G256_STAMP(10);
        }
    } else
    for (int t = 0; t < nk; ++t) {
        char* cur = smem + (t & 1) * KBUF_BYTES;
        char* nxt = smem + ((t + 1) & 1) * KBUF_BYTES;
        const int k1 = kbeg + (t + 1) * BKT, k2 = kbeg + (t + 2) * BKT;
        const bool has1 = t + 1 < nk, has2 = t + 2 < nk;
        load_a(cur + OFF_A0);
        G256_LOAD_B(fb0, cur + OFF_B0);
        if (has1) stage_half<AK, 0, KTAIL>(p.A, p.lda, m0, p.M, k1, p.K, 1, nxt + OFF_A1, wave, lane);
        G256_WAIT_DMA(has2);
        G256_END_LOAD();
        G256_MFMA(0, 0, fb0);
        G256_END_MFMA();
        G256_LOAD_B(fb1, cur + OFF_B1);
        if (has2) stage_half<AK, 0, KTAIL>(p.A, p.lda, m0, p.M, k2, p.K, 0, cur + OFF_A0, wave, lane);
        G256_WAIT_DMA(has2);
        G256_END_LOAD();
        G256_MFMA(0, 1, fb1);
        G256_END_MFMA();
        load_a(cur + OFF_A1);
        if (has2) stage_half<BK, 1, KTAIL>(p.B, p.ldb, n0, p.N, k2, p.K, 0, cur + OFF_B0, wave, lane);
        G256_END_LOAD();
        G256_MFMA(1, 1, fb1);
        G256_END_MFMA();
        if (has2) stage_half<BK, 1, KTAIL>(p.B, p.ldb, n0, p.N, k2, p.K, 1, cur + OFF_B1, wave, lane);
        G256_WAIT_DMA(has2);
        G256_END_LOAD();
        G256_MFMA(1, 0, fb0);
        G256_END_MFMA();
    }
    if (wm == 0) {
        __builtin_amdgcn_s_barrier();
        __builtin_amdgcn_sched_barrier(0);
    }
    __syncthreads();
    G256_TSTAMP(2);
    G256_RSTAMP(6);

    if constexpr (kDirectOuts<Epi> > 0) {
        constexpr int NO = kDirectOuts<Epi>, DLD = 520;
        constexpr int ROWS = NO == 1 ? 256 : 128, NPASS = 256 / ROWS;
        const int nout = epi.n_direct();
        const int dcol = tid & 31, dgn = n0 + dcol * 8;
#pragma unroll
        for (int pass = 0; pass < NPASS; ++pass) {
#pragma unroll
            for (int half = 0; half < 2; ++half) {
                if (NO > 1 && half != pass) continue;
#pragma unroll
                for (int i = 0; i < 4; ++i)
#pragma unroll
                    for (int j = 0; j < 4; ++j) {
                        const int R = (NO == 1 ? half * 128 : 0) + wm * 64 + i * 16 + (lane & 15);
                        const int cb = (wn * 64 + j * 16 + 4 * (lane >> 4)) * 2;
                        u32x2_t o[NO];
                        epi.pw(acc[half * 4 + i][j], o, nout);
#pragma unroll
                        for (int w = 0; w < NO; ++w)
                            if (w < nout) *(u32x2_t*)(smem + w * (ROWS * DLD) + R * DLD + cb) = o[w];
                    }
            }
            __syncthreads();
#pragma unroll
            for (int it = 0; it < ROWS / 16; ++it) {
                const int R = (tid >> 5) + 16 * it;
                const int half = NO == 1 ? (R >> 7) : pass, row = R & 127;
                const int gm = m0 + (row >> 6) * 128 + half * 64 + (row & 63);
                if (gm < p.M && dgn < p.N) {
#pragma unroll
                    for (int w = 0; w < NO; ++w)
                        if (w < nout) {
                            const char* src = smem + w * (ROWS * DLD) + R * DLD + dcol * 16;
                            const u32x2_t lo = *(const u32x2_t*)src, hi = *(const u32x2_t*)(src + 8);
                            store16_stream(epi.dst(w) + (size_t)gm * epi.ldo + dgn, u32x4_t{lo.x, lo.y, hi.x, hi.y}, epi.keep_direct());
                        }
                }
            }
            if (pass + 1 < NPASS) __syncthreads();
        }
        G256_TSTAMP(3);
        G256_TSTAMP(4);
        G256_STAMPS_OUT();
        return;
    }
    if constexpr (kReduce<Epi>) {
        float* cs = (float*)smem;
        const int ecol = (tid & 31) * 8, gn = n0 + ecol;
        const bool col_ok = gn < p.N;
        float ck, ckb, ckd;
        epi.coef(ck, ckb, ckd);
        float gain_acc = 0.f;
        float tot[2][2][3];
        typename Epi::Aux aux[4];
#pragma unroll
        for (int pass = 0; pass < 2; ++pass) {
#pragma unroll
            for (int i = 0; i < 4; ++i)
#pragma unroll
                for (int j = 0; j < 4; ++j) {
                    const int row = wm * 64 + i * 16 + (lane & 15);
                    const int col = wn * 64 + j * 16 + 4 * (lane >> 4);
                    *(f32x4_t*)(cs + row * CS2_LD + col) = acc[pass * 4 + i][j];
                }
            typename Epi::Acc r;
            float* const red0 = (float*)(smem + SMEM2_BYTES);
            float* const red = (float*)smem;
#pragma unroll
            for (int half = 0; half < 2; ++half) {
                const int mb = m0 + half * 128 + pass * 64;
                typename Epi::Tile tl;
                const bool blk_ok = col_ok && mb < p.M;
                if (blk_ok) tl = epi.block_begin(mb, gn);
                if (pass == 0 && half == 0) {
#pragma unroll
                    for (int q = 0; q < 4; ++q) {
                        const int gm = mb + (tid >> 5) + 16 * q;
                        if (blk_ok && gm < p.M) aux[q] = epi.load(gm, gn);
                    }
                }
                if (half == 0) __syncthreads();
#pragma unroll
                for (int i = 0; i < 8; ++i) r.sc[i] = r.sh[i] = r.g[i] = 0.f;
                r.gain = 0.f;
                const int mb_next = half == 0 ? mb + 128 : m0 + 64;
                const bool next_ok = !(pass == 1 && half == 1) && col_ok && mb_next < p.M;
#pragma unroll
                for (int q = 0; q < 4; ++q) {
                    const int row = half * 64 + (tid >> 5) + 16 * q;
                    const int gm = mb + (tid >> 5) + 16 * q;
                    if (blk_ok && gm < p.M) {
                        float v[8];
                        *(f32x4_t*)(v) = *(const f32x4_t*)(cs + row * CS2_LD + ecol);
                        *(f32x4_t*)(v + 4) = *(const f32x4_t*)(cs + row * CS2_LD + ecol + 4);
                        epi.apply_r(gm, gn, v, aux[q], tl, r, ck, ckb, ckd);
                    }
                    const int gmn = mb_next + (tid >> 5) + 16 * q;
                    if (next_ok && gmn < p.M) aux[q] = epi.load(gmn, gn);
                }
                gain_acc += r.gain;
#pragma unroll
                for (int i = 0; i < 8; ++i) {
                    r.sc[i] += __shfl_xor(r.sc[i], 32, 64);
                    r.sh[i] += __shfl_xor(r.sh[i], 32, 64);
                    r.g[i] += __shfl_xor(r.g[i], 32, 64);
                }
                if (half == 1) __syncthreads();
                if (lane < 32) {
                    float* base = (half == 0 ? red0 : red) + wave * 256 + ecol;
                    *(float4*)(base) = make_float4(r.sc[0], r.sc[1], r.sc[2], r.sc[3]);
                    *(float4*)(base + 4) = make_float4(r.sc[4], r.sc[5], r.sc[6], r.sc[7]);
                    *(float4*)(base + 8 * 256) = make_float4(r.sh[0], r.sh[1], r.sh[2], r.sh[3]);
                    *(float4*)(base + 8 * 256 + 4) = make_float4(r.sh[4], r.sh[5], r.sh[6], r.sh[7]);
                    *(float4*)(base + 16 * 256) = make_float4(r.g[0], r.g[1], r.g[2], r.g[3]);
                    *(float4*)(base + 16 * 256 + 4) = make_float4(r.g[4], r.g[5], r.g[6], r.g[7]);
                }
            }
            __syncthreads();
            if (tid < 256) {
#pragma unroll
                for (int half = 0; half < 2; ++half)
#pragma unroll
                    for (int o = 0; o < 3; ++o) {
                        const float* src = half == 0 ? red0 : red;
                        float a = 0.f;
#pragma unroll
                        for (int w = 0; w < 8; ++w) a += src[(o * 8 + w) * 256 + tid];
                        tot[pass][half][o] = a;
                    }
            }
            __syncthreads();
        }
        if (tid < 256 && n0 + tid < p.N) {
            const int c = n0 + tid;
            int s_prev = -1;
            float a[3] = {0.f, 0.f, 0.f};
            auto flush = [&](int smp) {
                epi.dscale[(size_t)smp * epi.ldd + c] = a[0];
                epi.dshift[(size_t)smp * epi.ldd + c] = a[1];
                if (epi.y_up) epi.dg_up[(size_t)smp * epi.ldd_up + c] = a[2];
            };
#pragma unroll
            for (int b = 0; b < 4; ++b) {
                const int half = b >> 1, pass = b & 1;
                const int mb = m0 + 64 * b;
                if (mb < p.M) {
                    const int smp = mb / epi.T;
                    if (smp != s_prev) {
                        if (s_prev >= 0) flush(s_prev);
                        a[0] = a[1] = a[2] = 0.f;
                        s_prev = smp;
                    }
#pragma unroll
                    for (int o = 0; o < 3; ++o) a[o] += tot[pass][half][o];
                }
            }
            if (s_prev >= 0) flush(s_prev);
        }
        gain_acc = wave_sum(gain_acc);
        float* gred = (float*)smem;
        if (lane == 0) gred[wave] = gain_acc;
        __syncthreads();
        if (tid == 0) {
            float a = 0.f;
#pragma unroll
            for (int w = 0; w < 8; ++w) a += gred[w];
            epi.dgain_part[z * p.tiles + tile] = a * epi.gscale;
        }
        G256_STAMPS_OUT();
        return;
    } else {
    float* cs = (float*)smem;
    const int ecol = (tid & 31) * 8, gn = n0 + ecol;
    const bool col_ok = gn < p.N;
    typename Epi::Tile tctx;
    if (col_ok) tctx = epi.tile_begin(m0, (m0 + BM2 <= p.M ? m0 + BM2 : p.M) - 1, gn);
    unsigned uoff = 0;
    if constexpr (kUniformRows<Epi>) uoff = (unsigned)((tid >> 5) * epi.ld_rows() + ecol);
    constexpr bool IN = FE;
    typename Epi::Aux aux[8];
#pragma unroll
    for (int pass = 0; pass < 2; ++pass) {
#pragma unroll
        for (int i = 0; i < 4; ++i)
#pragma unroll
            for (int j = 0; j < 4; ++j) {
                const int row = wm * 64 + i * 16 + (lane & 15);
                const int col = wn * 64 + j * 16 + 4 * (lane >> 4);
                *(f32x4_t*)(cs + row * CS2_LD + col) = acc[pass * 4 + i][j];
            }
        if (pass == 0) {
#pragma unroll
            for (int it = 0; it < 8; ++it) {
                const int row = (tid >> 5) + 16 * it;
                const int gm = m0 + (row >> 6) * 128 + (row & 63);
                if constexpr (IN && kUniformRows<Epi>) aux[it] = epi_load_u(epi, m0 + (it >> 2) * 128 + (it & 3) * 16, n0, uoff);
                else if (IN || (gm < p.M && col_ok)) aux[it] = epi.load(gm, gn);
            }
        }
        __syncthreads();
#pragma unroll
        for (int it = 0; it < 8; ++it) {
            const int row = (tid >> 5) + 16 * it;
            const int gm = m0 + (row >> 6) * 128 + pass * 64 + (row & 63);
            if (IN || (gm < p.M && col_ok)) {
                float v[8];
                *(f32x4_t*)(v) = *(const f32x4_t*)(cs + row * CS2_LD + ecol);
                *(f32x4_t*)(v + 4) = *(const f32x4_t*)(cs + row * CS2_LD + ecol + 4);
                if constexpr (IN && kUniformRows<Epi>) epi_apply_u(epi, m0 + (it >> 2) * 128 + pass * 64 + (it & 3) * 16, n0, uoff, v, z, aux[it], tctx);
                else epi_apply_t<IN>(epi, gm, gn, v, z, aux[it], tctx);
            }
            if constexpr (IN && kUniformRows<Epi>) { if (pass == 0) aux[it] = epi_load_u(epi, m0 + (it >> 2) * 128 + 64 + (it & 3) * 16, n0, uoff); }
            else if (pass == 0 && (IN || (gm + 64 < p.M && col_ok))) aux[it] = epi.load(gm + 64, gn);
            if (IN) __builtin_amdgcn_sched_barrier(0);
        }
        __syncthreads();
        G256_TSTAMP(3 + pass);
    }
    G256_STAMPS_OUT();
    }
}

__device__ __forceinline__ void stagger_start(const GemmP& p) {
    const int pop = p.stagger >= 100 ? ((blockIdx.x >> 3) & 3) : ((blockIdx.x >> 3) & 1);
    const int n = (p.stagger >= 100 ? p.stagger - 100 : p.stagger) * pop;
    for (int i = 0; i < n; ++i) __builtin_amdgcn_s_sleep(127);
}

template <int AK, int BK, class Epi, bool KTAIL = false, bool FE = false>
__global__ __launch_bounds__(512, 2) void gemm_mfma256_kernel(GemmP p, Epi epi) {
#ifdef MAPDIT_GEMM_STAMPS
    __shared__ __attribute__((aligned(16))) char smem[SMEM2_BYTES + (2 * STAMP_TILES * STAMP_POINTS + 8) * 8];
#else
    __shared__ __attribute__((aligned(16))) char smem[kReduce<Epi> ? SMEM2_BYTES + 3 * 8 * 256 * 4 : SMEM2_BYTES];
#endif
    const int total = p.tiles * p.split_k;
    stagger_start(p);
    for (int v = blockIdx.x; v < total; v += gridDim.x) {
        gemm256_tile<AK, BK, Epi, KTAIL, FE>(p, epi, smem, v, total);
        __syncthreads();
    }
}

constexpr int GROUP_MAX = 4;
struct GroupArgs {
    GemmP p[GROUP_MAX];
    EpiStoreF32 e[GROUP_MAX];
    int first[GROUP_MAX + 1];
    int n;
};
__global__ __launch_bounds__(512, 2) void gemm_mfma256_group_kernel(GroupArgs g) {
#ifdef MAPDIT_GEMM_STAMPS
    __shared__ __attribute__((aligned(16))) char smem[SMEM2_BYTES + (2 * STAMP_TILES * STAMP_POINTS + 8) * 8];
#else
    __shared__ __attribute__((aligned(16))) char smem[SMEM2_BYTES];
#endif
    const int total = g.first[g.n];
    for (int v = blockIdx.x; v < total; v += gridDim.x) {
        int i = 0;
        while (i + 1 < g.n && v >= g.first[i + 1]) ++i;
        gemm256_tile<OP_KMAJ, OP_KMAJ, EpiStoreF32, false, false>(g.p[i], g.e[i], smem, v - g.first[i], g.first[i + 1] - g.first[i]);
        __syncthreads();
    }
}

struct TileCoord { int m0, n0, z, tile, kbeg, nk; };
__device__ __forceinline__ TileCoord tile_coord(const GemmP& p, const int bid, const int nwg) {
    const int xcd = bid & 7, q = nwg >> 3, r = nwg & 7;
    const int wg = (xcd < r ? xcd * (q + 1) : r * (q + 1) + (xcd - r) * q) + (bid >> 3);
    TileCoord c;
    c.z = wg / p.tiles;
    c.tile = wg - c.z * p.tiles;
    const int tiles_m = p.tiles / p.tiles_n;
    const int bsz = tiles_m * p.band;
    const int bidx = c.tile / bsz, rem = c.tile - bidx * bsz;
    const int bw = (bidx + 1) * p.band <= p.tiles_n ? p.band : p.tiles_n - bidx * p.band;
    c.m0 = (rem / bw) * BM2;
    c.n0 = (bidx * p.band + rem % bw) * BN2;
    const int nkt = (p.K + BKT - 1) / BKT, kbase = nkt / p.split_k, krem = nkt % p.split_k;
    c.kbeg = (c.z * kbase + (c.z < krem ? c.z : krem)) * BKT;
    c.nk = kbase + (c.z < krem ? 1 : 0);
    return c;
}

constexpr int WPRIV_BYTES = 4096;
constexpr int SMEM_W_BYTES = 2 * KBUF_BYTES + 8 * WPRIV_BYTES;

template <int AK, int BK, bool KTAIL>
__device__ __forceinline__ void g256_prologue(const GemmP& p, const TileCoord& c, char* smem, int wave, int lane) {
    stage_half<AK, 0, KTAIL>(p.A, p.lda, c.m0, p.M, c.kbeg, p.K, 0, smem + OFF_A0, wave, lane);
    stage_half<BK, 1, KTAIL>(p.B, p.ldb, c.n0, p.N, c.kbeg, p.K, 0, smem + OFF_B0, wave, lane);
    stage_half<BK, 1, KTAIL>(p.B, p.ldb, c.n0, p.N, c.kbeg, p.K, 1, smem + OFF_B1, wave, lane);
    stage_half<AK, 0, KTAIL>(p.A, p.lda, c.m0, p.M, c.kbeg, p.K, 1, smem + OFF_A1, wave, lane);
    if (c.nk > 1) {
        char* b1 = smem + KBUF_BYTES;
        stage_half<AK, 0, KTAIL>(p.A, p.lda, c.m0, p.M, c.kbeg + BKT, p.K, 0, b1 + OFF_A0, wave, lane);
        stage_half<BK, 1, KTAIL>(p.B, p.ldb, c.n0, p.N, c.kbeg + BKT, p.K, 0, b1 + OFF_B0, wave, lane);
        stage_half<BK, 1, KTAIL>(p.B, p.ldb, c.n0, p.N, c.kbeg + BKT, p.K, 1, b1 + OFF_B1, wave, lane);
    }
}

#ifndef MAPDIT_EPI_PD_AUX
#define MAPDIT_EPI_PD_AUX 2
#endif
template <class Epi> constexpr bool kWaveEpilogue = true;
template <class Epi> constexpr bool kWaveEpilogueAnyK = true;
template <> constexpr bool kWaveEpilogue<EpiResid> = false;
template <> constexpr bool kWaveEpilogue<EpiStoreF32> = false;
template <> constexpr bool kWaveEpilogueAnyK<EpiStoreBf16> = false;
template <class Epi> constexpr int kEpiPrefetch = 2;
template <class Epi> constexpr bool kEpiPipeline = true;
template <> constexpr int kEpiPrefetch<EpiResid> = 1;
template <> constexpr int kEpiPrefetch<EpiMulAux> = MAPDIT_EPI_PD_AUX;
template <> constexpr int kEpiPrefetch<EpiDSilu> = MAPDIT_EPI_PD_AUX;
template <> constexpr bool kEpiPipeline<EpiResid> = false;
template <class Epi, bool INTERIOR>
__device__ __forceinline__ void g256w_epilogue(const GemmP& p, const Epi& epi, const TileCoord& c, f32x4_t (&acc)[8][4],
                                               char* priv, const int wave, const int lane) {
    const int wm = wave >> 2, wn = wave & 3;
    const int cch = lane & 7, rsub = lane >> 3;
    const int wrow = lane & 15, wq = lane >> 4;
    const int gn = c.n0 + wn * 64 + cch * 8;
    const bool col_ok = INTERIOR || gn < p.N;
    typename Epi::Tile tctx;
    if (col_ok) tctx = epi.tile_begin(c.m0, (c.m0 + BM2 <= p.M ? c.m0 + BM2 : p.M) - 1, gn);
    f32x4_t* b = (f32x4_t*)priv;
    constexpr int PD = kEpiPrefetch<Epi>;
    constexpr bool PIPE = kEpiPipeline<Epi>;
    typename Epi::Aux aux[8][2];
    const int mw = c.m0 + wm * 128 + rsub;
    auto row_of = [&](int r, int s) { return mw + (r >> 2) * 64 + (r & 3) * 16 + 8 * s; };
    int woff[4], roff[2][2];
#pragma unroll
    for (int j = 0; j < 4; ++j) woff[j] = wrow * 16 + ((4 * j + wq) ^ (wrow & 7));
#pragma unroll
    for (int s = 0; s < 2; ++s) {
        const int rr = rsub + 8 * s;
        roff[s][0] = rr * 16 + ((2 * cch) ^ (rr & 7));
        roff[s][1] = rr * 16 + ((2 * cch + 1) ^ (rr & 7));
    }
#pragma unroll
    for (int r = 0; r < PD; ++r)
#pragma unroll
        for (int s = 0; s < 2; ++s)
            if (INTERIOR || (row_of(r, s) < p.M && col_ok)) aux[r][s] = epi.load(row_of(r, s), gn);
    f32x4_t cur[2][2], nxt[2][2];
    if (PIPE) {
#pragma unroll
        for (int j = 0; j < 4; ++j) b[woff[j]] = acc[0][j];
#pragma unroll
        for (int s = 0; s < 2; ++s) { cur[s][0] = b[roff[s][0]]; cur[s][1] = b[roff[s][1]]; }
    }
#pragma unroll
    for (int r = 0; r < 8; ++r) {
        if (r + PD < 8) {
#pragma unroll
            for (int s = 0; s < 2; ++s)
                if (INTERIOR || (row_of(r + PD, s) < p.M && col_ok)) aux[r + PD][s] = epi.load(row_of(r + PD, s), gn);
        }
        if (PIPE && r + 1 < 8) {
#pragma unroll
            for (int j = 0; j < 4; ++j) b[woff[j]] = acc[r + 1][j];
#pragma unroll
            for (int s = 0; s < 2; ++s) { nxt[s][0] = b[roff[s][0]]; nxt[s][1] = b[roff[s][1]]; }
        }
        if (!PIPE) {
#pragma unroll
            for (int j = 0; j < 4; ++j) b[woff[j]] = acc[r][j];
#pragma unroll
            for (int s = 0; s < 2; ++s) { cur[s][0] = b[roff[s][0]]; cur[s][1] = b[roff[s][1]]; }
        }
#pragma unroll
        for (int s = 0; s < 2; ++s) {
            float v[8];
            *(f32x4_t*)(v) = cur[s][0];
            *(f32x4_t*)(v + 4) = cur[s][1];
            if (INTERIOR || (row_of(r, s) < p.M && col_ok)) epi.apply(row_of(r, s), gn, v, c.z, aux[r][s], tctx);
        }
        if (PIPE) {
#pragma unroll
            for (int s = 0; s < 2; ++s) { cur[s][0] = nxt[s][0]; cur[s][1] = nxt[s][1]; }
        }
    }
}

template <int AK, int BK, class Epi, bool KTAIL = false>
__global__ __launch_bounds__(512, 2) void gemm_mfma256w_kernel(GemmP p, Epi epi) {
    __shared__ __attribute__((aligned(16))) char smem[SMEM_W_BYTES];
    const int total = p.tiles * p.split_k;
    int v = blockIdx.x;
    if (v >= total) return;
    stagger_start(p);
    constexpr bool TR_ASM2 = AK == OP_KMAJ;
    TileCoord c = tile_coord(p, v, total);
    {
        const int tid0 = threadIdx.x;
        g256_prologue<AK, BK, KTAIL>(p, c, smem, __builtin_amdgcn_readfirstlane(tid0 >> 6), tid0 & 63);
    }
    bool first = true;
#ifdef MAPDIT_GEMM_STAMPS
    long long ph_[4] = {0, 0, 0, 0};
    int ph_tiles_ = 0;
#define GW_STAMP(VAR) __builtin_amdgcn_sched_barrier(0); const long long VAR = (long long)__builtin_readcyclecounter(); __builtin_amdgcn_sched_barrier(0)
#else
#define GW_STAMP(VAR)
#endif
    for (;;) {
        int tid_ = threadIdx.x;
        asm volatile("" : "+v"(tid_));
        const int tid = tid_, lane = tid & 63;
        const int wave = __builtin_amdgcn_readfirstlane(tid >> 6);
        const int wm = wave >> 2, wn = wave & 3;
        const int m0 = c.m0, n0 = c.n0, kbeg = c.kbeg, nk = c.nk;
        f32x4_t acc[8][4];
#pragma unroll
        for (int i = 0; i < 8; ++i)
#pragma unroll
            for (int j = 0; j < 4; ++j) acc[i][j] = f32x4_t{0.f, 0.f, 0.f, 0.f};
        bf16x8_t fa[4][2], fb0[2][2], fb1[2][2];
        auto load_a = [&](const char* slot) {
#pragma unroll
            for (int i = 0; i < 4; ++i)
#pragma unroll
                for (int ks = 0; ks < 2; ++ks) fa[i][ks] = read_frag<AK, TR_ASM2>(slot, wm * 64 + i * 16, ks, lane);
        };
        GW_STAMP(ts0_);
        if (first && nk > 1) asm volatile("s_waitcnt vmcnt(8)" ::: "memory");
        else asm volatile("s_waitcnt vmcnt(0)" ::: "memory");
        __builtin_amdgcn_sched_barrier(0);
        __builtin_amdgcn_s_barrier();
        __builtin_amdgcn_sched_barrier(0);
        if (wm == 1) {
            __builtin_amdgcn_s_barrier();
            __builtin_amdgcn_sched_barrier(0);
        }
        GW_STAMP(ts1_);
        for (int t = 0; t < nk; ++t) {
            char* cur = smem + (t & 1) * KBUF_BYTES;
            char* nxt = smem + ((t + 1) & 1) * KBUF_BYTES;
            const int k1 = kbeg + (t + 1) * BKT, k2 = kbeg + (t + 2) * BKT;
            const bool has1 = t + 1 < nk, has2 = t + 2 < nk;
            load_a(cur + OFF_A0);
            G256_LOAD_B(fb0, cur + OFF_B0);
            G256_LOAD_B(fb1, cur + OFF_B1);
            if (has1) {
                stage_half<AK, 0, KTAIL>(p.A, p.lda, m0, p.M, k1, p.K, 1, nxt + OFF_A1, wave, lane);
                asm volatile("s_waitcnt vmcnt(8)" ::: "memory");
            } else {
                asm volatile("s_waitcnt vmcnt(0)" ::: "memory");
            }
            G256_END_LOAD();
            G256_MFMA(0, 0, fb0);
            G256_MFMA(0, 1, fb1);
            G256_END_MFMA();
            load_a(cur + OFF_A1);
            if (has2) {
                stage_half<AK, 0, KTAIL>(p.A, p.lda, m0, p.M, k2, p.K, 0, cur + OFF_A0, wave, lane);
                stage_half<BK, 1, KTAIL>(p.B, p.ldb, n0, p.N, k2, p.K, 0, cur + OFF_B0, wave, lane);
                stage_half<BK, 1, KTAIL>(p.B, p.ldb, n0, p.N, k2, p.K, 1, cur + OFF_B1, wave, lane);
                asm volatile("s_waitcnt vmcnt(8)" ::: "memory");
            } else if (has1) {
                asm volatile("s_waitcnt vmcnt(2)" ::: "memory");
            } else {
                asm volatile("s_waitcnt vmcnt(0)" ::: "memory");
            }
            G256_END_LOAD();
            G256_MFMA(1, 1, fb1);
            G256_MFMA(1, 0, fb0);
            G256_END_MFMA();
        }
        if (wm == 0) {
            __builtin_amdgcn_s_barrier();
            __builtin_amdgcn_sched_barrier(0);
        }
        GW_STAMP(ts2_);
        const int vn = v + (int)gridDim.x;
        TileCoord cn = c;
        if (vn < total) {
            cn = tile_coord(p, vn, total);
            g256_prologue<AK, BK, KTAIL>(p, cn, smem, wave, lane);
        }
        GW_STAMP(ts3_);
        if (c.m0 + BM2 <= p.M && c.n0 + BN2 <= p.N)
            g256w_epilogue<Epi, true>(p, epi, c, acc, smem + 2 * KBUF_BYTES + wave * WPRIV_BYTES, wave, lane);
        else
            g256w_epilogue<Epi, false>(p, epi, c, acc, smem + 2 * KBUF_BYTES + wave * WPRIV_BYTES, wave, lane);
#ifdef MAPDIT_GEMM_STAMPS
        {
            GW_STAMP(ts4_);
            ph_[0] += ts1_ - ts0_; ph_[1] += ts2_ - ts1_; ph_[2] += ts3_ - ts2_; ph_[3] += ts4_ - ts3_;
            ++ph_tiles_;
            if ((vn >= total) && g_wg_times && (wave & 3) == 0 && lane == 0) {
                long long* r_ = g_wg_times + 16 * (long long)blockIdx.x + 8 * (wave >> 2);
                r_[0] = ph_[0]; r_[1] = ph_[1]; r_[2] = ph_[2]; r_[3] = ph_[3]; r_[4] = ph_tiles_;
            }
        }
#endif
        if (vn >= total) break;
        v = vn;
        c = cn;
        first = false;
    }
}

template <class Epi>
__global__ void gemm_simple_kernel(const bf16_t* __restrict__ A, long sam, long sak, const bf16_t* __restrict__ B,
                                   long sbn, long sbk, int M, int N, int K, Epi epi) {
    const int chunks = N >> 3;
    const long id = (long)blockIdx.x * blockDim.x + threadIdx.x;
    if (id >= (long)M * chunks) return;
    const int m = (int)(id / chunks), n = (int)(id % chunks) * 8;
    float v[8] = {0, 0, 0, 0, 0, 0, 0, 0};
    for (int k = 0; k < K; ++k) {
        const float a = up16(A[m * sam + k * sak]);
#pragma unroll
        for (int i = 0; i < 8; ++i) v[i] += a * up16(B[(n + i) * sbn + k * sbk]);
    }
    epi(m, n, v);
}

MD_NS_CLOSE

#ifdef MAPDIT_GEMM_STAMPS
extern "C" void mapdit_debug_set_stamps(long long* p) {
    hipLaunchKernelGGL(mapdit_debug_set_stamps_kernel, dim3(1), dim3(1), 0, 0, p, -1);
    (void)hipDeviceSynchronize();
}
extern "C" void mapdit_debug_set_wg_times(long long* p) {
    hipLaunchKernelGGL(mapdit_debug_set_wg_times_kernel, dim3(1), dim3(1), 0, 0, p);
    (void)hipDeviceSynchronize();
}
extern "C" void mapdit_debug_set_stamps_block(long long* p, int block) {
    hipLaunchKernelGGL(mapdit_debug_set_stamps_kernel, dim3(1), dim3(1), 0, 0, p, block);
    (void)hipDeviceSynchronize();
}
#endif

static int gemm_phases_arg(int v) { return v == 4 || v == 6 || v == 7 ? v : 2; }

struct GemmEnv {
    int tile = 0;
    int phases = 2;
    long band = 0;
    int old_tile_rule = 0;
    int persist = 256;
    int keep_mask = 1;
    int nsplit = 1;
    int fast_epi = 1;
    int band768 = 3;
    int stagger = -1;
    GemmEnv() {
        if (const char* e = getenv("MAPDIT_GEMM_PERSIST")) persist = atoi(e);
        if (const char* e = getenv("MAPDIT_KEEP")) keep_mask = atoi(e);
        if (const char* e = getenv("MAPDIT_GEMM_NSPLIT")) nsplit = atoi(e);
        if (const char* e = getenv("MAPDIT_GEMM_STAGGER")) stagger = atoi(e);
        if (const char* e = getenv("MAPDIT_GEMM_BAND768")) band768 = atoi(e) > 0 ? atoi(e) : 3;
        if (const char* e = getenv("MAPDIT_GEMM_FE")) fast_epi = atoi(e);
        if (const char* e = getenv("MAPDIT_GEMM_TILE_RULE")) old_tile_rule = e[0] == 'o';
        if (const char* e = getenv("MAPDIT_GEMM_TILE")) tile = atoi(e);
        if (const char* e = getenv("MAPDIT_GEMM_PHASES")) phases = gemm_phases_arg(atoi(e));
        if (const char* e = getenv("MAPDIT_GEMM_BAND")) band = atol(e);
    }
};
GemmEnv& mapdit_gemm_env_ref();
static GemmEnv& gemm_env() { return mapdit_gemm_env_ref(); }
#if MAPDIT_DT == 0
GemmEnv& mapdit_gemm_env_ref() {
    static GemmEnv env;
    return env;
}
extern "C" void mapdit_gemm_tuning(int tile, int phases, long band) {
    GemmEnv& e = gemm_env();
    e.tile = tile;
    e.phases = gemm_phases_arg(phases);
    e.band = band;
}

extern "C" int mapdit_gemm_tile_size_k(int M, int N, int K, int split_k_launch) {
    const int force = gemm_env().tile;
    if (force == 128 || force == 256) return force;
    if (!(M >= 512 && N >= 256)) return 128;
    const long t256 = (long)cdiv(M, 256) * cdiv(N, 256);
    if (split_k_launch) {
        if (t256 < 12) return 128;
        if (!gemm_env().old_tile_rule && (double)M * N < 0.85 * (double)t256 * 65536.0) return 128;
        if (K > 0 && !gemm_env().old_tile_rule) {
            const long slabs = 256 / t256 > 0 ? 256 / t256 : 1;
            if ((K / 64) / slabs < 24) return 128;
        }
        return 256;
    }
    if (t256 < 128) return 128;
    if (!gemm_env().old_tile_rule && t256 > 256 && t256 <= 320) return 128;
    return 256;
}
extern "C" int mapdit_gemm_tile_size_ex(int M, int N, int split_k_launch) { return mapdit_gemm_tile_size_k(M, N, 0, split_k_launch); }
extern "C" int mapdit_gemm_tile_size(int M, int N) { return mapdit_gemm_tile_size_ex(M, N, 0); }
#endif

MD_NS_OPEN

template <class Epi> constexpr bool kHasTail = false;
template <> constexpr bool kHasTail<EpiStoreF32> = true;

template <class F>
inline void with_operand_kinds(int layout, F&& f) {
    using Row = std::integral_constant<int, OP_ROW>;
    using Kmaj = std::integral_constant<int, OP_KMAJ>;
    if (layout == MAPDIT_NT) f(Row(), Row());
    else if (layout == MAPDIT_NN) f(Row(), Kmaj());
    else f(Kmaj(), Kmaj());
}

template <class Epi>
int launch(int layout, int M, int N, int K, const bf16_t* A, int lda, const bf16_t* B, int ldb, Epi epi,
           hipStream_t st, int split_k = 1, int n_off = 0, bool force128 = false) {
    bool a_kmaj = false, b_kmaj = false;
    with_operand_kinds(layout, [&](auto ak, auto bk) { a_kmaj = ak.value == OP_KMAJ; b_kmaj = bk.value == OP_KMAJ; });
    if constexpr (!kReduce<Epi>) {
        if (!force128 && n_off == 0 && split_k == 1 && gemm_env().nsplit && N % 256 == 128 && N >= 384 && K % BKT == 0 &&
            gemm_env().tile != 128 && M >= 512 && (long)cdiv(M, 256) * ((N - 128) / 256) >= 192 &&
            (long)cdiv(M, 256) * ((N - 128) / 256) <= 256 && !(((uintptr_t)A | (uintptr_t)B) & 15) &&
            lda % 8 == 0 && ldb % 8 == 0 && !(a_kmaj && M % 8 != 0)) {
            const int N1 = N - 128;
            const bf16_t* B2 = b_kmaj ? B + N1 : B + (size_t)N1 * ldb;
            if (!(((uintptr_t)B2) & 15)) {
                const int rc = launch(layout, M, N1, K, A, lda, B, ldb, epi, st, 1, 0, false);
                if (rc != MAPDIT_OK) return rc;
                return launch(layout, M, 128, K, A, lda, B2, ldb, epi, st, 1, N1, true);
            }
        }
    }
    const bool ktail = K % BKT != 0;
    bool mfma = (K % 8 == 0) && (N % 8 == 0) && K > 0 && (!ktail || kHasTail<Epi>);
    if (a_kmaj && (M % 8 != 0 || lda % 8 != 0)) mfma = false;
    if (b_kmaj && (ldb % 8 != 0)) mfma = false;
    if (!a_kmaj && lda % 8 != 0) mfma = false;
    if (!b_kmaj && ldb % 8 != 0) mfma = false;
    if (((uintptr_t)A | (uintptr_t)B) & 15) mfma = false;
    if constexpr (kReduce<Epi>) {
        if (!mfma || ktail || mapdit_gemm_tile_size_k(M, N, K, 0) != 256) {
            mapdit_set_error("gemm: this epilogue needs the 256x256 MFMA path (M=%d N=%d K=%d: K %% 64 == 0, M >= 512, N >= 256, aligned operands)", M, N, K);
            return MAPDIT_ERR_ARG;
        }
    }
    if (split_k > 1 && (!mfma || split_k > (K + BKT - 1) / BKT)) {
        mapdit_set_error("gemm: split_k=%d needs the MFMA path and split_k <= ceil(K/64) (K=%d)", split_k, K);
        return MAPDIT_ERR_ARG;
    }
    if (mfma && !force128 && mapdit_gemm_tile_size_k(M, N, K, split_k > 1) == 256) {
        GemmP p{A, B, lda, ldb, M, N, K, cdiv(N, BN2), 0, split_k, 0, 2, 0, 0};
        p.tiles = cdiv(M, BM2) * p.tiles_n;
        p.phases = gemm_env().phases;
        const bool be = gemm_env().band > 0;
        long band = be ? gemm_env().band : (long)(2.5 * 1024 * 1024) / ((long)BN2 * (K / split_k) * 2);
        if (!be && band < 4) band = p.tiles_n;
        if (!be && layout == MAPDIT_NT && split_k == 1 && K <= 768 && p.tiles_n >= 6 && p.tiles_n % gemm_env().band768 == 0) band = gemm_env().band768;
        if (band < 1 || band > p.tiles_n) band = p.tiles_n;
        p.band = (int)band;
        int grid = p.tiles * split_k;
        if (gemm_env().persist && grid >= 3 * gemm_env().persist) {
            grid = gemm_env().persist;
            const int sg = gemm_env().stagger;
            p.stagger = sg >= 0 ? sg : (std::is_same<Epi, EpiResid>::value ? 2 : 0);
        }
        bool use_w = false;
        if constexpr (!kReduce<Epi>)
            use_w = p.phases == 6 || (p.phases == 2 && kWaveEpilogue<Epi> && (kWaveEpilogueAnyK<Epi> || K / split_k <= 1024));
        if (p.phases == 7 || p.phases == 6) p.phases = 2;
        bool fe = false;
        if constexpr (kFastEpi<Epi>)
            fe = gemm_env().fast_epi && M % BM2 == 0 && N % BN2 == 0 && epi.fast_ok();
        auto go = [&](auto tail) {
            constexpr bool TAIL = decltype(tail)::value;
            with_operand_kinds(layout, [&](auto ak, auto bk) {
                if constexpr (!kReduce<Epi>) {
                    if (use_w) { hipLaunchKernelGGL((gemm_mfma256w_kernel<ak.value, bk.value, Epi, TAIL>), dim3(grid), dim3(512), 0, st, p, epi); return; }
                }
                if constexpr (kFastEpi<Epi> && !TAIL) {
                    if (fe) { hipLaunchKernelGGL((gemm_mfma256_kernel<ak.value, bk.value, Epi, false, true>), dim3(grid), dim3(512), 0, st, p, epi); return; }
                }
                hipLaunchKernelGGL((gemm_mfma256_kernel<ak.value, bk.value, Epi, TAIL>), dim3(grid), dim3(512), 0, st, p, epi);
            });
        };
        if constexpr (kHasTail<Epi>) {
            if (ktail) {
                go(std::true_type());
                MD_LAUNCH_CHECK();
                return MAPDIT_OK;
            }
        }
        go(std::false_type());
    } else if (mfma) {
        if constexpr (std::is_same<Epi, EpiResid>::value || std::is_same<Epi, EpiStoreBf16>::value) {
            static const bool t64_env = [] { const char* v = getenv("MAPDIT_GEMM_TILE64"); return !(v && v[0] == '0'); }();
            const long t128 = (long)cdiv(M, BM) * cdiv(N, BN);
            if (t64_env && !a_kmaj && !ktail && split_k == 1 && t128 <= 160 && M >= 256) {
                GemmP p{A, B, lda, ldb, M, N, K, cdiv(N, BN), 0, 1, 0, 4, n_off, 0};
                p.tiles = cdiv(M, 64) * p.tiles_n;
                with_operand_kinds(layout, [&](auto, auto bk) {
                    hipLaunchKernelGGL((gemm_mfma64_kernel<bk.value, Epi>), dim3(p.tiles), dim3(256), 0, st, p, epi);
                });
                MD_LAUNCH_CHECK();
                return MAPDIT_OK;
            }
        }
        GemmP p{A, B, lda, ldb, M, N, K, cdiv(N, BN), 0, split_k, 0, 4, n_off, 0};
        p.tiles = cdiv(M, BM) * p.tiles_n;
        const int grid = p.tiles * split_k;
        if constexpr (kHasTail<Epi>) {
            if (ktail) {
                with_operand_kinds(layout, [&](auto ak, auto bk) {
                    hipLaunchKernelGGL((gemm_mfma_kernel<ak.value, bk.value, Epi, true>), dim3(grid), dim3(256), 0, st, p, epi);
                });
                MD_LAUNCH_CHECK();
                return MAPDIT_OK;
            }
        }
        with_operand_kinds(layout, [&](auto ak, auto bk) {
            hipLaunchKernelGGL((gemm_mfma_kernel<ak.value, bk.value, Epi>), dim3(grid), dim3(256), 0, st, p, epi);
        });
    } else {
        if (n_off != 0 || force128) {
            mapdit_set_error("gemm: internal: column-offset launch reached the non-MFMA path (M=%d N=%d K=%d)", M, N, K);
            return MAPDIT_ERR_ARG;
        }
        const long sam = a_kmaj ? 1 : lda, sak = a_kmaj ? lda : 1;
        const long sbn = b_kmaj ? 1 : ldb, sbk = b_kmaj ? ldb : 1;
        const long total = (long)M * (N >> 3);
        hipLaunchKernelGGL((gemm_simple_kernel<Epi>), dim3(cdiv(total, 256)), dim3(256), 0, st, A, sam, sak, B, sbn, sbk, M, N, K, epi);
    }
    MD_LAUNCH_CHECK();
    return MAPDIT_OK;
}

MD_NS_CLOSE

#if MAPDIT_DT == 0
static thread_local char g_err[512] = "";
void mapdit_set_error(const char* fmt, ...) {
    va_list ap;
    va_start(ap, fmt);
    vsnprintf(g_err, sizeof(g_err), fmt, ap);
    va_end(ap);
}
extern "C" const char* mapdit_last_error(void) { return g_err; }
extern "C" int mapdit_abi_version(void) { return 5; }
#endif

extern "C" int MD_SYM_GEMM_GROUP(int n, const mapdit_gemm_group_item_t* items, int K, int split_k, void* stream) {
    MD_CHECK(items && n >= 1 && n <= GROUP_MAX, "gemm_group: 1..%d items", GROUP_MAX);
    MD_CHECK(K > 0 && K % BKT == 0 && split_k >= 1 && split_k <= K / BKT, "gemm_group: K=%d must be a multiple of 64 and split_k=%d <= K / 64", K, split_k);
    GroupArgs g{};
    g.n = n;
    for (int i = 0; i < n; ++i) {
        const mapdit_gemm_group_item_t& it = items[i];
        MD_CHECK(it.A && it.B && it.out && it.M > 0 && it.N > 0, "gemm_group: item %d: null / empty", i);
        MD_CHECK(it.M % 8 == 0 && it.N % 8 == 0 && it.lda % 8 == 0 && it.ldb % 8 == 0 && it.lda >= it.M && it.ldb >= it.N && it.ldo >= it.N && it.ldo % 4 == 0 &&
                 !(((uintptr_t)it.A | (uintptr_t)it.B | (uintptr_t)it.out) & 15),
                 "gemm_group: item %d is not on the MFMA path (M, N, lda, ldb multiples of 8; 16-byte aligned operands)", i);
        MD_CHECK(split_k == 1 || it.slab_stride >= (long)it.M * it.ldo, "gemm_group: item %d: slab_stride too small", i);
        GemmP& p = g.p[i];
        p.A = (const bf16_t*)it.A; p.B = (const bf16_t*)it.B; p.lda = it.lda; p.ldb = it.ldb; p.M = it.M; p.N = it.N; p.K = K;
        p.tiles_n = cdiv(it.N, BN2); p.tiles = cdiv(it.M, BM2) * p.tiles_n; p.split_k = split_k; p.phases = 2; p.n_off = 0; p.stagger = 0;
        long band = (long)(2.5 * 1024 * 1024) / ((long)BN2 * (K / split_k) * 2);
        if (band < 4 || band > p.tiles_n) band = p.tiles_n;
        p.band = (int)band;
        g.e[i] = EpiStoreF32{it.out, it.ldo, it.alpha, 0, it.slab_stride};
        g.first[i + 1] = g.first[i] + p.tiles * split_k;
    }
    hipLaunchKernelGGL(gemm_mfma256_group_kernel, dim3(g.first[n]), dim3(512), 0, (hipStream_t)stream, g);
    MD_LAUNCH_CHECK();
    return MAPDIT_OK;
}

extern "C" int MD_SYM_GEMM(int layout, int M, int N, int K, const uint16_t* A, int lda, const uint16_t* B,
                                int ldb, const mapdit_epilogue_t* e, void* stream) {
    MD_CHECK(layout >= MAPDIT_NT && layout <= MAPDIT_TN, "gemm: bad layout %d", layout);
    MD_CHECK(M > 0 && N > 0 && K > 0 && A && B && e, "gemm: null/empty argument (M=%d N=%d K=%d)", M, N, K);
    MD_CHECK(e->out || e->kind == MAPDIT_EPI_SILU2 || e->kind == MAPDIT_EPI_SILU2_COND || e->kind == MAPDIT_EPI_RESID ||
                 e->kind == MAPDIT_EPI_SILU2_GRAD || e->kind == MAPDIT_EPI_RMB,
             "gemm: null output");
    MD_CHECK(N % 8 == 0, "gemm: N=%d must be a multiple of 8", N);
    MD_CHECK(e->ldo % 8 == 0 || e->kind == MAPDIT_EPI_QKV_HEADS, "gemm: ldo=%d must be a multiple of 8", e->ldo);
    hipStream_t st = (hipStream_t)stream;
    MD_CHECK(e->split_k <= 1 || e->kind == MAPDIT_EPI_STORE_F32, "gemm: split_k is only available with EPI_STORE_F32");
    switch (e->kind) {
        case MAPDIT_EPI_STORE_BF16:
            return launch(layout, M, N, K, A, lda, B, ldb, EpiStoreBf16{(bf16_t*)e->out, e->ldo, e->alpha, (gemm_env().keep_mask >> 1) & 1}, st);
        case MAPDIT_EPI_STORE_F32:
            MD_CHECK(e->split_k <= 1 || !e->accumulate, "gemm: split_k with accumulate is not supported");
            return launch(layout, M, N, K, A, lda, B, ldb,
                          EpiStoreF32{(float*)e->out, e->ldo, e->alpha, e->accumulate, e->slab_stride}, st,
                          e->split_k > 1 ? e->split_k : 1);
        case MAPDIT_EPI_SILU2:
            MD_CHECK(e->out2, "gemm: SILU2 needs out2");
            return launch(layout, M, N, K, A, lda, B, ldb, EpiSilu2<0>{(bf16_t*)e->out, (bf16_t*)e->out2, e->ldo}, st);
        case MAPDIT_EPI_SILU2_COND:
            MD_CHECK(e->out2, "gemm: SILU2 needs out2");
            return launch(layout, M, N, K, A, lda, B, ldb, EpiSilu2<1>{(bf16_t*)e->out, (bf16_t*)e->out2, e->ldo}, st);
        case MAPDIT_EPI_RESID:
            MD_CHECK(e->out2 && e->aux && e->gate && e->rows_per_sample > 0, "gemm: RESID needs out2, aux, gate, rows_per_sample");
            MD_CHECK(e->ldg % 4 == 0, "gemm: ldg=%d must be a multiple of 4", e->ldg);
            MD_CHECK(!e->out3 || (e->shift2 && e->scale2 && (e->gain2 || e->rot2) && e->ld2 % 4 == 0),
                     "gemm: RESID fused modulate needs shift2, scale2, gain2 (unless rot2), ld2 %% 4 == 0");
            return launch(layout, M, N, K, A, lda, B, ldb,
                          EpiResid{(bf16_t*)e->out, (const float*)e->aux, (float*)e->out2, e->gate, e->ldo, e->ldg,
                                   e->rows_per_sample, e->alpha, e->beta, (bf16_t*)e->out3, e->shift2, e->scale2, e->gain2,
                                   e->ld2, e->rot2, (gemm_env().keep_mask & 1) | ((gemm_env().keep_mask >> 5) & 1) << 1}, st);
        case MAPDIT_EPI_SILU2_GRAD:
            MD_CHECK(e->out2, "gemm: SILU2_GRAD needs out2");
            if (e->out) return launch(layout, M, N, K, A, lda, B, ldb, EpiSilu2GradT<true>{(bf16_t*)e->out, (bf16_t*)e->out2, e->ldo, (gemm_env().keep_mask >> 3) & 1}, st);
            return launch(layout, M, N, K, A, lda, B, ldb, EpiSilu2GradT<false>{(bf16_t*)e->out, (bf16_t*)e->out2, e->ldo, (gemm_env().keep_mask >> 3) & 1}, st);
        case MAPDIT_EPI_MUL_AUX:
            MD_CHECK(e->aux, "gemm: MUL_AUX needs aux");
            return launch(layout, M, N, K, A, lda, B, ldb, EpiMulAux{(bf16_t*)e->out, (const bf16_t*)e->aux, e->ldo, (gemm_env().keep_mask >> 4) & 1}, st);
        case MAPDIT_EPI_DSILU:
            MD_CHECK(e->aux, "gemm: DSILU needs aux (pre-activation)");
            return launch(layout, M, N, K, A, lda, B, ldb, EpiDSilu{(bf16_t*)e->out, (const bf16_t*)e->aux, e->ldo}, st);
        case MAPDIT_EPI_RMB: {
            const mapdit_resid_mod_bwd_t* a = (const mapdit_resid_mod_bwd_t*)e->rmb;
            MD_CHECK(a, "gemm: RMB needs rmb");
            MD_CHECK(a->x && a->shift && a->scale && a->gain && a->dshift && a->dscale && a->dgain_part && (a->dx || a->dx_bf),
                     "gemm: RMB needs x, shift, scale, gain, dshift, dscale, dgain_part and dx or dx_bf");
            MD_CHECK(!a->y_up || (a->g_up && a->dy_up && a->dg_up), "gemm: RMB residual backward needs g_up, dy_up, dg_up");
            MD_CHECK(!a->rot, "gemm: the RMB epilogue computes the AdaLN form only (rot != 0: use mapdit_resid_mod_bwd after a plain dX GEMM)");
            MD_CHECK(a->T > 0 && a->T % 64 == 0 && 256 % a->T == 0 && M % a->T == 0 && (N == a->D || (N < a->D && N % 256 == 0 && e->ldo >= a->D)),
                     "gemm: RMB needs T in {64, 128, 256}, M = samples * T, N = D or a multiple of 256 below it (T=%d M=%d N=%d D=%d)", a->T, M, N, a->D);
            MD_CHECK(a->ldmod % 4 == 0 && a->ldg_up % 4 == 0 && e->ldo % 8 == 0, "gemm: RMB row strides must be multiples of 4 / 8");
            MD_CHECK(!(a->dxo && a->dxo_bf), "gemm: RMB: dxo and dxo_bf are alternatives");
            if (a->dxo_bf && a->dx_bf && a->y_up && !a->dx)
                return launch(layout, M, N, K, A, lda, B, ldb,
                              EpiRmbT<true, true>{(const bf16_t*)a->dxo_bf, nullptr, a->x, a->shift, a->scale, a->gain, (const bf16_t*)a->y_up, a->g_up, nullptr,
                                                  (bf16_t*)a->dx_bf, (bf16_t*)a->dy_up, a->dshift, a->dscale, a->dg_up, a->dgain_part, e->ldo, a->ldmod,
                                                  a->ldg_up, a->ldd, a->ldd_up, a->T, a->ca, a->cb, a->dgain_scale != 0.f ? a->dgain_scale : 1.f}, st);
            if (a->dxo_bf)
                return launch(layout, M, N, K, A, lda, B, ldb,
                              EpiRmbT<true>{(const bf16_t*)a->dxo_bf, nullptr, a->x, a->shift, a->scale, a->gain, (const bf16_t*)a->y_up, a->g_up, a->dx,
                                            (bf16_t*)a->dx_bf, (bf16_t*)a->dy_up, a->dshift, a->dscale, a->dg_up, a->dgain_part, e->ldo, a->ldmod,
                                            a->ldg_up, a->ldd, a->ldd_up, a->T, a->ca, a->cb, a->dgain_scale != 0.f ? a->dgain_scale : 1.f}, st);
            return launch(layout, M, N, K, A, lda, B, ldb,
                          EpiRmbT<false>{nullptr, a->dxo, a->x, a->shift, a->scale, a->gain, (const bf16_t*)a->y_up, a->g_up, a->dx, (bf16_t*)a->dx_bf,
                                         (bf16_t*)a->dy_up, a->dshift, a->dscale, a->dg_up, a->dgain_part, e->ldo, a->ldmod, a->ldg_up, a->ldd,
                                         a->ldd_up, a->T, a->ca, a->cb, a->dgain_scale != 0.f ? a->dgain_scale : 1.f}, st);
        }
        case MAPDIT_EPI_QKV_HEADS: {
            MD_CHECK(e->out2 && e->out3 && e->out4 && e->rows_per_sample > 0, "gemm: QKV_HEADS needs out2, out3, out4, rows_per_sample");
            MD_CHECK(N % 192 == 0 && M % e->rows_per_sample == 0, "gemm: QKV_HEADS needs N = 3 * 64 * heads, M = samples * rows_per_sample");
            const int H = N / 192;
            return launch(layout, M, N, K, A, lda, B, ldb,
                          EpiQkvHeads{(gemm_env().keep_mask >> 2) & 1, (bf16_t*)e->out, (bf16_t*)e->out2, (bf16_t*)e->out3, (float*)e->out4, e->rows_per_sample, H,
                                      (long)M * H,
                                      (e->rows_per_sample & (e->rows_per_sample - 1)) == 0 ? __builtin_ctz(e->rows_per_sample) : -1}, st);
        }
        case MAPDIT_EPI_QKV_HEADS_RAW: {
            const int hd = e->ld2, T = e->rows_per_sample;
            MD_CHECK(e->out && e->out2 && e->out3 && T > 0 && hd > 0 && hd % 8 == 0, "gemm: QKV_HEADS_RAW needs out, out2, out3, rows_per_sample, ld2 = head_dim (multiple of 8)");
            MD_CHECK(N % (3 * hd) == 0 && M % T == 0, "gemm: QKV_HEADS_RAW needs N = 3 * head_dim * heads, M = samples * rows_per_sample");
            return launch(layout, M, N, K, A, lda, B, ldb,
                          EpiHeadsRaw{(bf16_t*)e->out, (bf16_t*)e->out2, (bf16_t*)e->out3, T, N / (3 * hd), hd,
                                      (T & (T - 1)) == 0 ? __builtin_ctz(T) : -1}, st);
        }
    }
    mapdit_set_error("gemm: unknown epilogue kind %d", e->kind);
    return MAPDIT_ERR_ARG;
}
```

Baseline: 5938 latent-img/s.

## Stage GEMM tiles with hand-written global_load_lds DMA on aligned shapes

Adds a fast path to the 64/128/256 MFMA GEMM kernels and the grouped TN kernel. When shapes divide the tile evenly and the operand extents fit 32-bit offsets, the generic stage_tile/stage_half loaders are replaced by inline-asm global_load_lds_dwordx4 sequences, using precomputed swizzled per-lane offsets and scalar base pointers that advance each k-step. This is meant to cut address arithmetic and VGPR round-trips when filling LDS. The cost is fragile inline asm that manipulates m0, plus extra vmcnt waits in the 128/64 kernels. It is enabled by default and can be disabled with MAPDIT_GEMM_DMA=0.

```diff
diff --git a/include/mapdit.h b/include/mapdit.h
--- a/include/mapdit.h
+++ b/include/mapdit.h
@@ -69,6 +69,8 @@
 int mapdit_gemm_tile_size_ex(int M, int N, int split_k_launch);
 int mapdit_gemm_tile_size_k(int M, int N, int K, int split_k_launch);
 void mapdit_gemm_tuning(int tile, int phases, long band);
+int mapdit_gemm_dma_fast(int layout, int M, int N, int K, int lda, int ldb, int tile);
+int mapdit_gemm_dma_extent_ok(long rows, long ld);
 
 enum { MAPDIT_WN_PLAIN = 2 };
 int mapdit_weightnorm_fwd(float* W, int rows, int cols, int forced, float out_scale, uint16_t* w_bf16, float* w_f32,
diff --git a/map-dit_amd/_lib.py b/map-dit_amd/_lib.py
--- a/map-dit_amd/_lib.py
+++ b/map-dit_amd/_lib.py
@@ -179,6 +179,8 @@
     "mapdit_gemm_tile_size_ex": (ci, [ci, ci, ci]),
     "mapdit_gemm_tile_size_k": (ci, [ci, ci, ci, ci]),
     "mapdit_gemm_tuning": (None, [ci, ci, cl]),
+    "mapdit_gemm_dma_fast": (ci, [ci, ci, ci, ci, ci, ci, ci]),
+    "mapdit_gemm_dma_extent_ok": (ci, [cl, cl]),
     "mapdit_engine_workspace_bytes": (C.c_size_t, [C.POINTER(Config), ci]),
     "mapdit_engine_destroy": (None, [vp]),
     "mapdit_comm_destroy": (None, [vp]),
diff --git a/map-dit_amd/csrc/gemm.hip b/map-dit_amd/csrc/gemm.hip
--- a/map-dit_amd/csrc/gemm.hip
+++ b/map-dit_amd/csrc/gemm.hip
@@ -530,7 +530,48 @@
     }
 };
 
-template <int AK, int BK, class Epi, bool KTAIL = false>
+__device__ __forceinline__ unsigned lds_addr(const char* q) { return (unsigned)(size_t)(const __attribute__((address_space(3))) char*)q; }
+
+#define DMA_PIECE_FIRST(V, B) "s_mov_b32 m0, %[dst]\n\ts_nop 4\n\tglobal_load_lds_dwordx4 %[" V "], %[" B "]\n\t"
+#define DMA_PIECE(OFF, V, B) "s_add_u32 m0, %[dst], " OFF "\n\ts_nop 0\n\tglobal_load_lds_dwordx4 %[" V "], %[" B "]\n\t"
+
+template <int KIND> struct DmaCtx128 {
+    const char* pos;
+    unsigned voff, voff2, dj, dk;
+    __device__ __forceinline__ void begin(const bf16_t* G, int ld, int idx0, int kbeg, int wave, int lane) {
+        const unsigned pitch = (unsigned)ld * 2u;
+        unsigned v0, v2;
+        if (KIND == OP_ROW) {
+            pos = (const char*)G + ((size_t)(idx0 + wave * 32) * ld + kbeg) * 2;
+            v0 = v2 = (unsigned)(lane >> 3) * pitch + (unsigned)(((lane & 7) ^ (lane >> 3)) << 4);
+            dj = 8u * pitch; dk = BKT * 2;
+        } else {
+            pos = (const char*)G + ((size_t)(kbeg + wave * 16) * ld + idx0) * 2;
+            v0 = (unsigned)(lane >> 4) * pitch + (unsigned)(((lane & 15) ^ ((lane >> 4) << 1)) << 4);
+            v2 = (unsigned)(lane >> 4) * pitch + (unsigned)(((lane & 15) ^ (((lane >> 4) | 4) << 1)) << 4);
+            dj = 4u * pitch; dk = BKT * pitch;
+        }
+        asm volatile("" : "+v"(v0), "+v"(v2));
+        voff = v0; voff2 = v2;
+    }
+    __device__ __forceinline__ void stage(char* tile, int wave) {
+        const char *b0 = pos, *b1 = pos + dj, *b2 = pos + 2 * (size_t)dj, *b3 = pos + 3 * (size_t)dj;
+        unsigned keep;
+        asm volatile("s_mov_b32 %[keep], m0\n\t"
+                     DMA_PIECE_FIRST("v0", "b0")
+                     DMA_PIECE("0x400", "v0", "b1")
+                     DMA_PIECE("0x800", "v2", "b2")
+                     DMA_PIECE("0xc00", "v2", "b3")
+                     "s_mov_b32 m0, %[keep]"
+                     : [keep] "=&s"(keep)
+                     : [v0] "v"(voff), [v2] "v"(voff2), [dst] "s"(lds_addr(tile + wave * 4096)), [b0] "s"(b0), [b1] "s"(b1), [b2] "s"(b2),
+                       [b3] "s"(b3)
+                     : "memory", "scc");
+        pos += dk;
+    }
+};
+
+template <int AK, int BK, class Epi, bool KTAIL = false, bool FAST = false>
 __global__ __launch_bounds__(256, 2) void gemm_mfma_kernel(GemmP p, Epi epi) {
     __shared__ __attribute__((aligned(16))) char smem[SMEM_BYTES];
     const int tid = threadIdx.x, lane = tid & 63;
@@ -552,16 +593,27 @@
         for (int j = 0; j < 4; ++j) acc[i][j] = f32x4_t{0.f, 0.f, 0.f, 0.f};
 
     const int nk = kbase + (z < krem ? 1 : 0);
-    stage_tile<AK, KTAIL>(p.A, p.lda, m0, p.M, kbeg, p.K, smem, wave, lane);
-    stage_tile<BK, KTAIL>(p.B, p.ldb, n0, p.N, kbeg, p.K, smem + TILE_BYTES, wave, lane);
+    DmaCtx128<AK> ca;
+    DmaCtx128<BK> cb;
+    if constexpr (FAST) {
+        ca.begin(p.A, p.lda, m0, kbeg, wave, lane);
+        cb.begin(p.B, p.ldb, n0, kbeg, wave, lane);
+    }
+    auto stage = [&](int t, char* buf) {
+        if constexpr (FAST) {
+            ca.stage(buf, wave);
+            cb.stage(buf + TILE_BYTES, wave);
+        } else {
+            stage_tile<AK, KTAIL>(p.A, p.lda, m0, p.M, kbeg + t * BKT, p.K, buf, wave, lane);
+            stage_tile<BK, KTAIL>(p.B, p.ldb, n0, p.N, kbeg + t * BKT, p.K, buf + TILE_BYTES, wave, lane);
+        }
+    };
+    stage(0, smem);
     for (int t = 0; t < nk; ++t) {
+        if constexpr (FAST) asm volatile("s_waitcnt vmcnt(0)" ::: "memory");
         __syncthreads();
         char* cur = smem + (t & 1) * BUF_BYTES;
-        if (t + 1 < nk) {
-            char* nxt = smem + ((t + 1) & 1) * BUF_BYTES;
-            stage_tile<AK, KTAIL>(p.A, p.lda, m0, p.M, kbeg + (t + 1) * BKT, p.K, nxt, wave, lane);
-            stage_tile<BK, KTAIL>(p.B, p.ldb, n0, p.N, kbeg + (t + 1) * BKT, p.K, nxt + TILE_BYTES, wave, lane);
-        }
+        if (t + 1 < nk) stage(t + 1, smem + ((t + 1) & 1) * BUF_BYTES);
 #pragma unroll
         for (int ks = 0; ks < 2; ++ks) {
             bf16x8_t fa[4], fb[4];
@@ -605,7 +657,7 @@
     }
 }
 
-template <int BK, class Epi>
+template <int BK, class Epi, bool FAST = false>
 __global__ __launch_bounds__(256, 2) void gemm_mfma64_kernel(GemmP p, Epi epi) {
     __shared__ __attribute__((aligned(16))) char smem[SMEM_BYTES];
     const int tid = threadIdx.x, lane = tid & 63;
@@ -620,16 +672,27 @@
     for (int i = 0; i < 4; ++i)
 #pragma unroll
         for (int j = 0; j < 2; ++j) acc[i][j] = f32x4_t{0.f, 0.f, 0.f, 0.f};
-    if (wave < 2) stage_tile<OP_ROW, false>(p.A, p.lda, m0, p.M, 0, p.K, smem, wave, lane);
-    stage_tile<BK, false>(p.B, p.ldb, n0, p.N, 0, p.K, smem + TILE_BYTES, wave, lane);
+    DmaCtx128<OP_ROW> ca;
+    DmaCtx128<BK> cb;
+    if constexpr (FAST) {
+        ca.begin(p.A, p.lda, m0, 0, wave, lane);
+        cb.begin(p.B, p.ldb, n0, 0, wave, lane);
+    }
+    auto stage = [&](int t, char* buf) {
+        if constexpr (FAST) {
+            if (wave < 2) ca.stage(buf, wave);
+            cb.stage(buf + TILE_BYTES, wave);
+        } else {
+            if (wave < 2) stage_tile<OP_ROW, false>(p.A, p.lda, m0, p.M, t * BKT, p.K, buf, wave, lane);
+            stage_tile<BK, false>(p.B, p.ldb, n0, p.N, t * BKT, p.K, buf + TILE_BYTES, wave, lane);
+        }
+    };
+    stage(0, smem);
     for (int t = 0; t < nk; ++t) {
+        if constexpr (FAST) asm volatile("s_waitcnt vmcnt(0)" ::: "memory");
         __syncthreads();
         char* cur = smem + (t & 1) * BUF_BYTES;
-        if (t + 1 < nk) {
-            char* nxt = smem + ((t + 1) & 1) * BUF_BYTES;
-            if (wave < 2) stage_tile<OP_ROW, false>(p.A, p.lda, m0, p.M, (t + 1) * BKT, p.K, nxt, wave, lane);
-            stage_tile<BK, false>(p.B, p.ldb, n0, p.N, (t + 1) * BKT, p.K, nxt + TILE_BYTES, wave, lane);
-        }
+        if (t + 1 < nk) stage(t + 1, smem + ((t + 1) & 1) * BUF_BYTES);
 #pragma unroll
         for (int ks = 0; ks < 2; ++ks) {
             bf16x8_t fa[4], fb[2];
@@ -760,6 +823,105 @@
     }
 }
 
+template <int KIND, int SIDE> struct DmaCtx {
+    static constexpr int HALF = SIDE == 0 ? 64 : 32;
+    const char* base;
+    unsigned voff;
+    unsigned voff1;
+    unsigned dh;
+    unsigned dk;
+    __device__ __forceinline__ void begin(const bf16_t* G, int ld, int idx0, int kbeg, int wave, int lane) {
+        const unsigned pitch = (unsigned)ld * 2u;
+        unsigned vo, dj;
+        if (KIND == OP_ROW) {
+            const int wrow = SIDE == 0 ? (wave >> 2) * 128 + (wave & 3) * 16 : (wave >> 1) * 64 + (wave & 1) * 16;
+            base = (const char*)G + ((size_t)(idx0 + wrow) * ld + kbeg) * 2;
+            vo = (unsigned)(lane >> 3) * pitch + (unsigned)(((lane & 7) ^ (lane >> 3)) << 4);
+            dj = 8u * pitch; dh = HALF * pitch; dk = BKT * 2;
+        } else {
+            const int c = (lane & 15) ^ (((lane >> 4) | ((wave & 1) << 2)) << 1);
+            base = (const char*)G + ((size_t)(kbeg + wave * 8) * ld + idx0) * 2;
+            vo = (unsigned)(lane >> 4) * pitch + (unsigned)half_map<SIDE>(c * 8, 0) * 2u;
+            dj = 4u * pitch; dh = HALF * 2; dk = BKT * pitch;
+        }
+        unsigned vo1 = vo + dj;
+        asm volatile("" : "+v"(vo), "+v"(vo1));
+        voff = vo; voff1 = vo1;
+    }
+    __device__ __forceinline__ const char* at(const char* pos, int rel, int h) const {
+        return pos + (size_t)rel * dk + (size_t)h * dh;
+    }
+};
+
+__device__ __forceinline__ void dma_half(unsigned v0, unsigned v1, unsigned dst, const char* b) {
+    unsigned keep;
+    asm volatile("s_mov_b32 %[keep], m0\n\t"
+                 DMA_PIECE_FIRST("v0", "b")
+                 DMA_PIECE("0x400", "v1", "b")
+                 "s_mov_b32 m0, %[keep]"
+                 : [keep] "=&s"(keep)
+                 : [v0] "v"(v0), [v1] "v"(v1), [dst] "s"(dst), [b] "s"(b)
+                 : "memory", "scc");
+}
+__device__ __forceinline__ void dma_a0b0b1(unsigned va0, unsigned va1, unsigned vb0, unsigned vb1, unsigned dst, const char* a,
+                                           const char* b0, const char* b1) {
+    static_assert(OFF_A0 == 0 && OFF_B0 == 0x8000 && OFF_B1 == 0xc000, "slot offsets are spelled out in the asm below");
+    unsigned keep;
+    asm volatile("s_mov_b32 %[keep], m0\n\t"
+                 DMA_PIECE_FIRST("va0", "a")
+                 DMA_PIECE("0x400", "va1", "a")
+                 DMA_PIECE("0x8000", "vb0", "b0")
+                 DMA_PIECE("0x8400", "vb1", "b0")
+                 DMA_PIECE("0xc000", "vb0", "b1")
+                 DMA_PIECE("0xc400", "vb1", "b1")
+                 "s_mov_b32 m0, %[keep]"
+                 : [keep] "=&s"(keep)
+                 : [va0] "v"(va0), [va1] "v"(va1), [vb0] "v"(vb0), [vb1] "v"(vb1), [dst] "s"(dst), [a] "s"(a), [b0] "s"(b0), [b1] "s"(b1)
+                 : "memory", "scc");
+}
+
+template <int AK, int BK, bool KTAIL, bool FAST> struct Stage256 {
+    const GemmP& p;
+    const int m0, n0, kbeg, wave, lane;
+    DmaCtx<AK, 0> ca;
+    DmaCtx<BK, 1> cb;
+    const char *pa, *pb;
+    __device__ __forceinline__ Stage256(const GemmP& p_, int m0_, int n0_, int kbeg_, int wave_, int lane_)
+        : p(p_), m0(m0_), n0(n0_), kbeg(kbeg_), wave(wave_), lane(lane_) {
+        if constexpr (FAST) {
+            ca.begin(p.A, p.lda, m0, kbeg, wave, lane);
+            cb.begin(p.B, p.ldb, n0, kbeg, wave, lane);
+            pa = ca.base; pb = cb.base;
+        }
+    }
+    __device__ __forceinline__ void next() {
+        if constexpr (FAST) { pa += ca.dk; pb += cb.dk; }
+    }
+    template <int H> __device__ __forceinline__ void half_a(int t, int rel, char* slot) const {
+        if constexpr (FAST) dma_half(ca.voff, ca.voff1, lds_addr(slot + wave * 2048), ca.at(pa, rel, H));
+        else stage_half<AK, 0, KTAIL>(p.A, p.lda, m0, p.M, kbeg + (t + rel) * BKT, p.K, H, slot, wave, lane);
+    }
+    template <int H> __device__ __forceinline__ void half_b(int t, int rel, char* slot) const {
+        if constexpr (FAST) dma_half(cb.voff, cb.voff1, lds_addr(slot + wave * 2048), cb.at(pb, rel, H));
+        else stage_half<BK, 1, KTAIL>(p.B, p.ldb, n0, p.N, kbeg + (t + rel) * BKT, p.K, H, slot, wave, lane);
+    }
+    __device__ __forceinline__ void a0b0b1(int t, int rel, char* buf) const {
+        if constexpr (FAST) {
+            dma_a0b0b1(ca.voff, ca.voff1, cb.voff, cb.voff1, lds_addr(buf + wave * 2048), ca.at(pa, rel, 0),
+                                            cb.at(pb, rel, 0), cb.at(pb, rel, 1));
+        } else {
+            half_a<0>(t, rel, buf + OFF_A0);
+            half_b<0>(t, rel, buf + OFF_B0);
+            half_b<1>(t, rel, buf + OFF_B1);
+        }
+    }
+    __device__ __forceinline__ void prologue(char* smem, int nk) const {
+        a0b0b1(0, 0, smem);
+        half_a<1>(0, 0, smem + OFF_A1);
+        if (nk > 1) a0b0b1(0, 1, smem + KBUF_BYTES);
+    }
+};
+
 #define G256_END_LOAD()                                   \
     asm volatile("s_waitcnt lgkmcnt(0)" ::: "memory");    \
     __builtin_amdgcn_sched_barrier(0);                    \
@@ -770,7 +932,7 @@
     __builtin_amdgcn_s_barrier();                         \
     __builtin_amdgcn_sched_barrier(0)
 
-template <int AK, int BK, class Epi, bool KTAIL, bool FE = false>
+template <int AK, int BK, class Epi, bool KTAIL, bool FE = false, bool FAST = false>
 __device__ __forceinline__ void gemm256_tile(const GemmP& p, const Epi& epi, char* smem, const int bid, const int nwg) {
 #ifdef MAPDIT_GEMM_STAMPS
     long long* stamp_lds = (long long*)(smem + SMEM2_BYTES);
@@ -829,15 +991,9 @@
     if (has2) asm volatile("s_waitcnt vmcnt(10)" ::: "memory");              \
     else asm volatile("s_waitcnt vmcnt(0)" ::: "memory")
 
-    stage_half<AK, 0, KTAIL>(p.A, p.lda, m0, p.M, kbeg, p.K, 0, smem + OFF_A0, wave, lane);
-    stage_half<BK, 1, KTAIL>(p.B, p.ldb, n0, p.N, kbeg, p.K, 0, smem + OFF_B0, wave, lane);
-    stage_half<BK, 1, KTAIL>(p.B, p.ldb, n0, p.N, kbeg, p.K, 1, smem + OFF_B1, wave, lane);
-    stage_half<AK, 0, KTAIL>(p.A, p.lda, m0, p.M, kbeg, p.K, 1, smem + OFF_A1, wave, lane);
+    Stage256<AK, BK, KTAIL, FAST> sg(p, m0, n0, kbeg, wave, lane);
+    sg.prologue(smem, nk);
     if (nk > 1) {
-        char* b1 = smem + KBUF_BYTES;
-        stage_half<AK, 0, KTAIL>(p.A, p.lda, m0, p.M, kbeg + BKT, p.K, 0, b1 + OFF_A0, wave, lane);
-        stage_half<BK, 1, KTAIL>(p.B, p.ldb, n0, p.N, kbeg + BKT, p.K, 0, b1 + OFF_B0, wave, lane);
-        stage_half<BK, 1, KTAIL>(p.B, p.ldb, n0, p.N, kbeg + BKT, p.K, 1, b1 + OFF_B1, wave, lane);
         if (p.phases == 2) asm volatile("s_waitcnt vmcnt(8)" ::: "memory");
         else asm volatile("s_waitcnt vmcnt(10)" ::: "memory");
     } else {
@@ -857,14 +1013,13 @@
         for (int t = 0; t < nk; ++t) {
             char* cur = smem + (t & 1) * KBUF_BYTES;
             char* nxt = smem + ((t + 1) & 1) * KBUF_BYTES;
-            const int k1 = kbeg + (t + 1) * BKT, k2 = kbeg + (t + 2) * BKT;
             const bool has1 = t + 1 < nk, has2 = t + 2 < nk;
             G256_STAMP(0);
             load_a(cur + OFF_A0);
             G256_LOAD_B(fb0, cur + OFF_B0);
             G256_LOAD_B(fb1, cur + OFF_B1);
             if (has1) {
-                stage_half<AK, 0, KTAIL>(p.A, p.lda, m0, p.M, k1, p.K, 1, nxt + OFF_A1, wave, lane);
+                sg.template half_a<1>(t, 1, nxt + OFF_A1);
                 G256_STAMP(1);
                 asm volatile("s_waitcnt vmcnt(8)" ::: "memory");
             } else {
@@ -880,9 +1035,7 @@
             G256_STAMP(5);
             load_a(cur + OFF_A1);
             if (has2) {
-                stage_half<AK, 0, KTAIL>(p.A, p.lda, m0, p.M, k2, p.K, 0, cur + OFF_A0, wave, lane);
-                stage_half<BK, 1, KTAIL>(p.B, p.ldb, n0, p.N, k2, p.K, 0, cur + OFF_B0, wave, lane);
-                stage_half<BK, 1, KTAIL>(p.B, p.ldb, n0, p.N, k2, p.K, 1, cur + OFF_B1, wave, lane);
+                sg.a0b0b1(t, 2, cur);
                 G256_STAMP(6);
                 asm volatile("s_waitcnt vmcnt(8)" ::: "memory");
             } else if (has1) {
@@ -898,36 +1051,37 @@
             G256_STAMP(9);
             G256_END_MFMA();
             G256_STAMP(10);
+            sg.next();
         }
     } else
     for (int t = 0; t < nk; ++t) {
         char* cur = smem + (t & 1) * KBUF_BYTES;
         char* nxt = smem + ((t + 1) & 1) * KBUF_BYTES;
-        const int k1 = kbeg + (t + 1) * BKT, k2 = kbeg + (t + 2) * BKT;
         const bool has1 = t + 1 < nk, has2 = t + 2 < nk;
         load_a(cur + OFF_A0);
         G256_LOAD_B(fb0, cur + OFF_B0);
-        if (has1) stage_half<AK, 0, KTAIL>(p.A, p.lda, m0, p.M, k1, p.K, 1, nxt + OFF_A1, wave, lane);
+        if (has1) sg.template half_a<1>(t, 1, nxt + OFF_A1);
         G256_WAIT_DMA(has2);
         G256_END_LOAD();
         G256_MFMA(0, 0, fb0);
         G256_END_MFMA();
         G256_LOAD_B(fb1, cur + OFF_B1);
-        if (has2) stage_half<AK, 0, KTAIL>(p.A, p.lda, m0, p.M, k2, p.K, 0, cur + OFF_A0, wave, lane);
+        if (has2) sg.template half_a<0>(t, 2, cur + OFF_A0);
         G256_WAIT_DMA(has2);
         G256_END_LOAD();
         G256_MFMA(0, 1, fb1);
         G256_END_MFMA();
         load_a(cur + OFF_A1);
-        if (has2) stage_half<BK, 1, KTAIL>(p.B, p.ldb, n0, p.N, k2, p.K, 0, cur + OFF_B0, wave, lane);
+        if (has2) sg.template half_b<0>(t, 2, cur + OFF_B0);
         G256_END_LOAD();
         G256_MFMA(1, 1, fb1);
         G256_END_MFMA();
-        if (has2) stage_half<BK, 1, KTAIL>(p.B, p.ldb, n0, p.N, k2, p.K, 1, cur + OFF_B1, wave, lane);
+        if (has2) sg.template half_b<1>(t, 2, cur + OFF_B1);
         G256_WAIT_DMA(has2);
         G256_END_LOAD();
         G256_MFMA(1, 0, fb0);
         G256_END_MFMA();
+        sg.next();
     }
     if (wm == 0) {
         __builtin_amdgcn_s_barrier();
@@ -1166,7 +1320,7 @@
     for (int i = 0; i < n; ++i) __builtin_amdgcn_s_sleep(127);
 }
 
-template <int AK, int BK, class Epi, bool KTAIL = false, bool FE = false>
+template <int AK, int BK, class Epi, bool KTAIL = false, bool FE = false, bool FAST = false>
 __global__ __launch_bounds__(512, 2) void gemm_mfma256_kernel(GemmP p, Epi epi) {
 #ifdef MAPDIT_GEMM_STAMPS
     __shared__ __attribute__((aligned(16))) char smem[SMEM2_BYTES + (2 * STAMP_TILES * STAMP_POINTS + 8) * 8];
@@ -1176,7 +1330,7 @@
     const int total = p.tiles * p.split_k;
     stagger_start(p);
     for (int v = blockIdx.x; v < total; v += gridDim.x) {
-        gemm256_tile<AK, BK, Epi, KTAIL, FE>(p, epi, smem, v, total);
+        gemm256_tile<AK, BK, Epi, KTAIL, FE, FAST>(p, epi, smem, v, total);
         __syncthreads();
     }
 }
@@ -1188,6 +1342,7 @@
     int first[GROUP_MAX + 1];
     int n;
 };
+template <bool FAST>
 __global__ __launch_bounds__(512, 2) void gemm_mfma256_group_kernel(GroupArgs g) {
 #ifdef MAPDIT_GEMM_STAMPS
     __shared__ __attribute__((aligned(16))) char smem[SMEM2_BYTES + (2 * STAMP_TILES * STAMP_POINTS + 8) * 8];
@@ -1198,7 +1353,7 @@
     for (int v = blockIdx.x; v < total; v += gridDim.x) {
         int i = 0;
         while (i + 1 < g.n && v >= g.first[i + 1]) ++i;
-        gemm256_tile<OP_KMAJ, OP_KMAJ, EpiStoreF32, false, false>(g.p[i], g.e[i], smem, v - g.first[i], g.first[i + 1] - g.first[i]);
+        gemm256_tile<OP_KMAJ, OP_KMAJ, EpiStoreF32, false, false, FAST>(g.p[i], g.e[i], smem, v - g.first[i], g.first[i + 1] - g.first[i]);
         __syncthreads();
     }
 }
@@ -1225,18 +1380,10 @@
 constexpr int WPRIV_BYTES = 4096;
 constexpr int SMEM_W_BYTES = 2 * KBUF_BYTES + 8 * WPRIV_BYTES;
 
-template <int AK, int BK, bool KTAIL>
+template <int AK, int BK, bool KTAIL, bool FAST>
 __device__ __forceinline__ void g256_prologue(const GemmP& p, const TileCoord& c, char* smem, int wave, int lane) {
-    stage_half<AK, 0, KTAIL>(p.A, p.lda, c.m0, p.M, c.kbeg, p.K, 0, smem + OFF_A0, wave, lane);
-    stage_half<BK, 1, KTAIL>(p.B, p.ldb, c.n0, p.N, c.kbeg, p.K, 0, smem + OFF_B0, wave, lane);
-    stage_half<BK, 1, KTAIL>(p.B, p.ldb, c.n0, p.N, c.kbeg, p.K, 1, smem + OFF_B1, wave, lane);
-    stage_half<AK, 0, KTAIL>(p.A, p.lda, c.m0, p.M, c.kbeg, p.K, 1, smem + OFF_A1, wave, lane);
-    if (c.nk > 1) {
-        char* b1 = smem + KBUF_BYTES;
-        stage_half<AK, 0, KTAIL>(p.A, p.lda, c.m0, p.M, c.kbeg + BKT, p.K, 0, b1 + OFF_A0, wave, lane);
-        stage_half<BK, 1, KTAIL>(p.B, p.ldb, c.n0, p.N, c.kbeg + BKT, p.K, 0, b1 + OFF_B0, wave, lane);
-        stage_half<BK, 1, KTAIL>(p.B, p.ldb, c.n0, p.N, c.kbeg + BKT, p.K, 1, b1 + OFF_B1, wave, lane);
-    }
+    Stage256<AK, BK, KTAIL, FAST> sg(p, c.m0, c.n0, c.kbeg, wave, lane);
+    sg.prologue(smem, c.nk);
 }
 
 #ifndef MAPDIT_EPI_PD_AUX
@@ -1323,7 +1470,7 @@
     }
 }
 
-template <int AK, int BK, class Epi, bool KTAIL = false>
+template <int AK, int BK, class Epi, bool KTAIL = false, bool FAST = false>
 __global__ __launch_bounds__(512, 2) void gemm_mfma256w_kernel(GemmP p, Epi epi) {
     __shared__ __attribute__((aligned(16))) char smem[SMEM_W_BYTES];
     const int total = p.tiles * p.split_k;
@@ -1334,7 +1481,7 @@
     TileCoord c = tile_coord(p, v, total);
     {
         const int tid0 = threadIdx.x;
-        g256_prologue<AK, BK, KTAIL>(p, c, smem, __builtin_amdgcn_readfirstlane(tid0 >> 6), tid0 & 63);
+        g256_prologue<AK, BK, KTAIL, FAST>(p, c, smem, __builtin_amdgcn_readfirstlane(tid0 >> 6), tid0 & 63);
     }
     bool first = true;
 #ifdef MAPDIT_GEMM_STAMPS
@@ -1350,7 +1497,8 @@
         const int tid = tid_, lane = tid & 63;
         const int wave = __builtin_amdgcn_readfirstlane(tid >> 6);
         const int wm = wave >> 2, wn = wave & 3;
-        const int m0 = c.m0, n0 = c.n0, kbeg = c.kbeg, nk = c.nk;
+        const int nk = c.nk;
+        Stage256<AK, BK, KTAIL, FAST> sg(p, c.m0, c.n0, c.kbeg, wave, lane);
         f32x4_t acc[8][4];
 #pragma unroll
         for (int i = 0; i < 8; ++i)
@@ -1377,13 +1525,12 @@
         for (int t = 0; t < nk; ++t) {
             char* cur = smem + (t & 1) * KBUF_BYTES;
             char* nxt = smem + ((t + 1) & 1) * KBUF_BYTES;
-            const int k1 = kbeg + (t + 1) * BKT, k2 = kbeg + (t + 2) * BKT;
             const bool has1 = t + 1 < nk, has2 = t + 2 < nk;
             load_a(cur + OFF_A0);
             G256_LOAD_B(fb0, cur + OFF_B0);
             G256_LOAD_B(fb1, cur + OFF_B1);
             if (has1) {
-                stage_half<AK, 0, KTAIL>(p.A, p.lda, m0, p.M, k1, p.K, 1, nxt + OFF_A1, wave, lane);
+                sg.template half_a<1>(t, 1, nxt + OFF_A1);
                 asm volatile("s_waitcnt vmcnt(8)" ::: "memory");
             } else {
                 asm volatile("s_waitcnt vmcnt(0)" ::: "memory");
@@ -1394,9 +1541,7 @@
             G256_END_MFMA();
             load_a(cur + OFF_A1);
             if (has2) {
-                stage_half<AK, 0, KTAIL>(p.A, p.lda, m0, p.M, k2, p.K, 0, cur + OFF_A0, wave, lane);
-                stage_half<BK, 1, KTAIL>(p.B, p.ldb, n0, p.N, k2, p.K, 0, cur + OFF_B0, wave, lane);
-                stage_half<BK, 1, KTAIL>(p.B, p.ldb, n0, p.N, k2, p.K, 1, cur + OFF_B1, wave, lane);
+                sg.a0b0b1(t, 2, cur);
                 asm volatile("s_waitcnt vmcnt(8)" ::: "memory");
             } else if (has1) {
                 asm volatile("s_waitcnt vmcnt(2)" ::: "memory");
@@ -1407,6 +1552,7 @@
             G256_MFMA(1, 1, fb1);
             G256_MFMA(1, 0, fb0);
             G256_END_MFMA();
+            sg.next();
         }
         if (wm == 0) {
             __builtin_amdgcn_s_barrier();
@@ -1417,7 +1563,7 @@
         TileCoord cn = c;
         if (vn < total) {
             cn = tile_coord(p, vn, total);
-            g256_prologue<AK, BK, KTAIL>(p, cn, smem, wave, lane);
+            g256_prologue<AK, BK, KTAIL, FAST>(p, cn, smem, wave, lane);
         }
         GW_STAMP(ts3_);
         if (c.m0 + BM2 <= p.M && c.n0 + BN2 <= p.N)
@@ -1487,6 +1633,7 @@
     int nsplit = 1;
     int fast_epi = 1;
     int band768 = 3;
+    int dma_fast = 1;
     int stagger = -1;
     GemmEnv() {
         if (const char* e = getenv("MAPDIT_GEMM_PERSIST")) persist = atoi(e);
@@ -1495,6 +1642,7 @@
         if (const char* e = getenv("MAPDIT_GEMM_STAGGER")) stagger = atoi(e);
         if (const char* e = getenv("MAPDIT_GEMM_BAND768")) band768 = atoi(e) > 0 ? atoi(e) : 3;
         if (const char* e = getenv("MAPDIT_GEMM_FE")) fast_epi = atoi(e);
+        if (const char* e = getenv("MAPDIT_GEMM_DMA")) dma_fast = atoi(e);
         if (const char* e = getenv("MAPDIT_GEMM_TILE_RULE")) old_tile_rule = e[0] == 'o';
         if (const char* e = getenv("MAPDIT_GEMM_TILE")) tile = atoi(e);
         if (const char* e = getenv("MAPDIT_GEMM_PHASES")) phases = gemm_phases_arg(atoi(e));
@@ -1503,6 +1651,7 @@
 };
 GemmEnv& mapdit_gemm_env_ref();
 static GemmEnv& gemm_env() { return mapdit_gemm_env_ref(); }
+extern "C" int mapdit_gemm_dma_fast(int layout, int M, int N, int K, int lda, int ldb, int tile);
 #if MAPDIT_DT == 0
 GemmEnv& mapdit_gemm_env_ref() {
     static GemmEnv env;
@@ -1532,6 +1681,17 @@
     if (t256 < 128) return 128;
     if (!gemm_env().old_tile_rule && t256 > 256 && t256 <= 320) return 128;
     return 256;
+}
+
+extern "C" int mapdit_gemm_dma_extent_ok(long rows, long ld) {
+    return rows > 0 && ld > 0 && ld < (1l << 31) && rows < (1l << 32) && (unsigned long)rows * (unsigned long)ld * 2ul < (1ul << 32);
+}
+extern "C" int mapdit_gemm_dma_fast(int layout, int M, int N, int K, int lda, int ldb, int tile) {
+    if (layout < MAPDIT_NT || layout > MAPDIT_TN || (tile != 256 && tile != 128 && tile != 64)) return 0;
+    const int tn = tile == 256 ? 256 : 128;
+    if (M <= 0 || N <= 0 || K <= 0 || M % tile != 0 || N % tn != 0 || K % 64 != 0) return 0;
+    const bool a_kmaj = layout == MAPDIT_TN, b_kmaj = layout != MAPDIT_NT;
+    return mapdit_gemm_dma_extent_ok(a_kmaj ? K : M, lda) && mapdit_gemm_dma_extent_ok(b_kmaj ? K : N, ldb);
 }
 extern "C" int mapdit_gemm_tile_size_ex(int M, int N, int split_k_launch) { return mapdit_gemm_tile_size_k(M, N, 0, split_k_launch); }
 extern "C" int mapdit_gemm_tile_size(int M, int N) { return mapdit_gemm_tile_size_ex(M, N, 0); }
@@ -1610,26 +1770,28 @@
         bool fe = false;
         if constexpr (kFastEpi<Epi>)
             fe = gemm_env().fast_epi && M % BM2 == 0 && N % BN2 == 0 && epi.fast_ok();
-        auto go = [&](auto tail) {
-            constexpr bool TAIL = decltype(tail)::value;
+        const bool fast = gemm_env().dma_fast && mapdit_gemm_dma_fast(layout, M, N, K, lda, ldb, 256);
+        auto go = [&](auto tail, auto fst) {
+            constexpr bool TAIL = decltype(tail)::value, FAST = decltype(fst)::value;
             with_operand_kinds(layout, [&](auto ak, auto bk) {
                 if constexpr (!kReduce<Epi>) {
-                    if (use_w) { hipLaunchKernelGGL((gemm_mfma256w_kernel<ak.value, bk.value, Epi, TAIL>), dim3(grid), dim3(512), 0, st, p, epi); return; }
+                    if (use_w) { hipLaunchKernelGGL((gemm_mfma256w_kernel<ak.value, bk.value, Epi, TAIL, FAST>), dim3(grid), dim3(512), 0, st, p, epi); return; }
                 }
                 if constexpr (kFastEpi<Epi> && !TAIL) {
-                    if (fe) { hipLaunchKernelGGL((gemm_mfma256_kernel<ak.value, bk.value, Epi, false, true>), dim3(grid), dim3(512), 0, st, p, epi); return; }
+                    if (fe) { hipLaunchKernelGGL((gemm_mfma256_kernel<ak.value, bk.value, Epi, false, true, FAST>), dim3(grid), dim3(512), 0, st, p, epi); return; }
                 }
-                hipLaunchKernelGGL((gemm_mfma256_kernel<ak.value, bk.value, Epi, TAIL>), dim3(grid), dim3(512), 0, st, p, epi);
+                hipLaunchKernelGGL((gemm_mfma256_kernel<ak.value, bk.value, Epi, TAIL, false, FAST>), dim3(grid), dim3(512), 0, st, p, epi);
             });
         };
         if constexpr (kHasTail<Epi>) {
             if (ktail) {
-                go(std::true_type());
+                go(std::true_type(), std::false_type());
                 MD_LAUNCH_CHECK();
                 return MAPDIT_OK;
             }
         }
-        go(std::false_type());
+        if (fast) go(std::false_type(), std::true_type());
+        else go(std::false_type(), std::false_type());
     } else if (mfma) {
         if constexpr (std::is_same<Epi, EpiResid>::value || std::is_same<Epi, EpiStoreBf16>::value) {
             static const bool t64_env = [] { const char* v = getenv("MAPDIT_GEMM_TILE64"); return !(v && v[0] == '0'); }();
@@ -1637,8 +1799,10 @@
             if (t64_env && !a_kmaj && !ktail && split_k == 1 && t128 <= 160 && M >= 256) {
                 GemmP p{A, B, lda, ldb, M, N, K, cdiv(N, BN), 0, 1, 0, 4, n_off, 0};
                 p.tiles = cdiv(M, 64) * p.tiles_n;
+                const bool fast = gemm_env().dma_fast && mapdit_gemm_dma_fast(layout, M, N, K, lda, ldb, 64);
                 with_operand_kinds(layout, [&](auto, auto bk) {
-                    hipLaunchKernelGGL((gemm_mfma64_kernel<bk.value, Epi>), dim3(p.tiles), dim3(256), 0, st, p, epi);
+                    if (fast) hipLaunchKernelGGL((gemm_mfma64_kernel<bk.value, Epi, true>), dim3(p.tiles), dim3(256), 0, st, p, epi);
+                    else hipLaunchKernelGGL((gemm_mfma64_kernel<bk.value, Epi>), dim3(p.tiles), dim3(256), 0, st, p, epi);
                 });
                 MD_LAUNCH_CHECK();
                 return MAPDIT_OK;
@@ -1656,8 +1820,10 @@
                 return MAPDIT_OK;
             }
         }
+        const bool fast = gemm_env().dma_fast && mapdit_gemm_dma_fast(layout, M, N, K, lda, ldb, 128);
         with_operand_kinds(layout, [&](auto ak, auto bk) {
-            hipLaunchKernelGGL((gemm_mfma_kernel<ak.value, bk.value, Epi>), dim3(grid), dim3(256), 0, st, p, epi);
+            if (fast) hipLaunchKernelGGL((gemm_mfma_kernel<ak.value, bk.value, Epi, false, true>), dim3(grid), dim3(256), 0, st, p, epi);
+            else hipLaunchKernelGGL((gemm_mfma_kernel<ak.value, bk.value, Epi>), dim3(grid), dim3(256), 0, st, p, epi);
         });
     } else {
         if (n_off != 0 || force128) {
@@ -1692,6 +1858,7 @@
     MD_CHECK(K > 0 && K % BKT == 0 && split_k >= 1 && split_k <= K / BKT, "gemm_group: K=%d must be a multiple of 64 and split_k=%d <= K / 64", K, split_k);
     GroupArgs g{};
     g.n = n;
+    bool fast = gemm_env().dma_fast != 0;
     for (int i = 0; i < n; ++i) {
         const mapdit_gemm_group_item_t& it = items[i];
         MD_CHECK(it.A && it.B && it.out && it.M > 0 && it.N > 0, "gemm_group: item %d: null / empty", i);
@@ -1707,8 +1874,10 @@
         p.band = (int)band;
         g.e[i] = EpiStoreF32{it.out, it.ldo, it.alpha, 0, it.slab_stride};
         g.first[i + 1] = g.first[i] + p.tiles * split_k;
-    }
-    hipLaunchKernelGGL(gemm_mfma256_group_kernel, dim3(g.first[n]), dim3(512), 0, (hipStream_t)stream, g);
+        fast = fast && mapdit_gemm_dma_fast(MAPDIT_TN, it.M, it.N, K, it.lda, it.ldb, 256);
+    }
+    if (fast) hipLaunchKernelGGL(gemm_mfma256_group_kernel<true>, dim3(g.first[n]), dim3(512), 0, (hipStream_t)stream, g);
+    else hipLaunchKernelGGL(gemm_mfma256_group_kernel<false>, dim3(g.first[n]), dim3(512), 0, (hipStream_t)stream, g);
     MD_LAUNCH_CHECK();
     return MAPDIT_OK;
 }
```

After: 6032 latent-img/s (median of 6 runs). +1.6%, better.
